# milos-agathon/forge3d

Hardware: AMD Instinct MI355X
Metric: Msamples/s (W*H*spp/s) at 1920x1080, 11616 spp (8 spp/frame x 1452 frames timed); SSIM vs golden (higher is better)
Workload: dtype f32

## Files before the change

forge3d_amd/_native.py:

```python
from __future__ import annotations

import ctypes as C
import os
from pathlib import Path

import numpy as np

_PKG = Path(__file__).resolve().parent
LIB_PATH = _PKG / "libf3dhip.so"

STATUS_OK, STATUS_VALUE, STATUS_RENDER, STATUS_UPLOAD, STATUS_DEVICE = 0, 1, 2, 3, 4
ABI_VERSION = 6
FRAMES_IN_FLIGHT_AUTO = 0xFFFFFFFF

_EARTH = {"flat": 0, "sphere": 1, "ellipsoid": 2, "wgs84": 2}
_REFRACTION = {"none": 0, "bennett": 1, "saemundsson": 2, "effective_radius": 3}


class Desc(C.Structure):
    _fields_ = [
        ("struct_size", C.c_uint32),
        ("heights", C.c_void_p), ("dem_width", C.c_uint32), ("dem_height", C.c_uint32),
        ("spacing_x", C.c_float), ("spacing_z", C.c_float), ("exaggeration", C.c_float),
        ("albedo", C.c_float * 3),
# ... 181 lines not shown


DRAPE_NEAREST, DRAPE_BILINEAR = 0, 1
DRAPE_DEVICE_POINTERS, DRAPE_NO_WAIT, DRAPE_PATCH = 4, 8, 16
DRAPE_MAX_SIDE = 16384
DRAPE_TEXEL_MAX = 65504.0


_P = C.POINTER
ABI = [
    ("f3d_terrain_ref_render", C.c_int, [_P(Desc), _P(Out), C.c_char_p, C.c_size_t]),
    ("f3d_session_create", C.c_int, [_P(Desc), _P(SessionOpts), _P(C.c_void_p), C.c_char_p, C.c_size_t]),
    ("f3d_session_destroy", None, [C.c_void_p]),
    ("f3d_session_enqueue_frames", C.c_int, [C.c_void_p, C.c_uint32, C.c_uint32, C.c_int32, C.c_char_p, C.c_size_t]),
    ("f3d_session_enqueue_trace", C.c_int, [C.c_void_p, C.c_uint32, C.c_uint32, C.c_char_p, C.c_size_t]),
    ("f3d_session_enqueue_merge", C.c_int, [C.c_void_p, C.c_uint32, C.c_int32, C.c_char_p, C.c_size_t]),
    ("f3d_session_set_accumulation", C.c_int, [C.c_void_p, C.c_void_p, C.c_char_p, C.c_size_t]),
    ("f3d_session_halo_export", C.c_int, [C.c_void_p, _P(HaloExport), C.c_char_p, C.c_size_t]),
    ("f3d_session_halo_connect", C.c_int, [C.c_void_p, C.c_int32, _P(HaloExport), C.c_char_p, C.c_size_t]),
    ("f3d_session_halo_probe", C.c_int, [C.c_void_p, C.c_int32, C.c_uint32, _P(C.c_uint32), C.c_char_p, C.c_size_t]),
    ("f3d_session_halo_status", C.c_int, [C.c_void_p, _P(C.c_uint32), C.c_char_p, C.c_size_t]),
    ("f3d_session_halo_stats", C.c_int, [C.c_void_p, _P(HaloStats), C.c_char_p, C.c_size_t]),
    ("f3d_session_enqueue_batch_strip", C.c_int, [C.c_void_p, C.c_uint32, C.c_uint32, C.c_int32, C.c_char_p, C.c_size_t]),
    ("f3d_session_frames_in_flight", C.c_uint32, [C.c_void_p]),
    ("f3d_session_retraced_pixels", C.c_int, [C.c_void_p, _P(C.c_uint64)]),
    ("f3d_session_trace_batch", C.c_uint32, [C.c_void_p, C.c_uint32, C.c_uint32]),
    ("f3d_session_window_stats", C.c_int, [C.c_void_p, _P(C.c_float), _P(C.c_int32), C.c_char_p, C.c_size_t]),
    ("f3d_scene_cache_limit", None, [C.c_uint32]),
    ("f3d_scene_cache_entries", C.c_uint32, []),
    ("f3d_wavefront_render", C.c_int, [C.c_void_p, C.c_uint32, C.c_uint32, C.c_uint32, C.c_uint32, C.c_uint32, C.c_int32,
                                       C.c_void_p, C.c_char_p, C.c_size_t]),
    ("f3d_aether_bake", C.c_int, [C.c_void_p, C.c_void_p, C.c_void_p, C.c_void_p, C.c_void_p, C.c_void_p, _P(C.c_double),
                                  C.c_char_p, C.c_size_t]),
    ("f3d_smoke_render", C.c_int, [C.c_void_p, C.c_void_p, C.c_void_p, C.c_void_p, _P(C.c_double), C.c_char_p, C.c_size_t]),
    ("f3d_smoke_step", C.c_int, [C.c_void_p, C.c_void_p, C.c_void_p, C.c_uint32, C.c_uint32, _P(C.c_double), C.c_char_p, C.c_size_t]),
    ("f3d_aether_reference_render", C.c_int, [C.c_void_p, C.c_void_p, C.c_char_p, C.c_size_t]),
    ("f3d_smoke_composite", C.c_int, [C.c_void_p, C.c_void_p, _P(C.c_double), C.c_char_p, C.c_size_t]),
    ("f3d_session_fingerprint", C.c_int, [C.c_void_p, C.c_void_p, C.c_uint32]),
    ("f3d_session_mesh_tree", C.c_int, [C.c_void_p, _P(C.c_uint32), C.c_void_p, C.c_size_t, C.c_void_p, C.c_size_t, C.c_char_p, C.c_size_t]),
    ("f3d_session_rearm", C.c_int, [C.c_void_p, _P(RearmDesc), C.c_char_p, C.c_size_t]),
    ("f3d_session_render", C.c_int, [C.c_void_p, _P(Out), C.c_char_p, C.c_size_t]),
    ("f3d_session_reaim", C.c_int, [C.c_void_p, _P(ReaimDesc), C.c_char_p, C.c_size_t]),
    ("f3d_session_remesh", C.c_int, [C.c_void_p, _P(RemeshDesc), C.c_char_p, C.c_size_t]),
    ("f3d_session_reterrain", C.c_int, [C.c_void_p, _P(ReterrainDesc), C.c_char_p, C.c_size_t]),
    ("f3d_session_query", C.c_int, [C.c_void_p, _P(QueryDesc), C.c_char_p, C.c_size_t]),
    ("f3d_session_raster", C.c_int, [C.c_void_p, _P(RasterDesc), C.c_char_p, C.c_size_t]),
    ("f3d_session_horizon", C.c_int, [C.c_void_p, _P(HorizonDesc), C.c_char_p, C.c_size_t]),
    ("f3d_session_irradiation", C.c_int, [C.c_void_p, _P(IrradiationDesc), C.c_char_p, C.c_size_t]),
    ("f3d_session_clearance", C.c_int, [C.c_void_p, _P(ClearanceDesc), C.c_char_p, C.c_size_t]),
    ("f3d_session_drape", C.c_int, [C.c_void_p, _P(DrapeDesc), C.c_char_p, C.c_size_t]),
    ("f3d_session_draped", C.c_int, [C.c_void_p, _P(C.c_uint32)]),
    ("f3d_session_certificates", C.c_int, [C.c_void_p, _P(C.c_uint64)]),
    ("f3d_session_sky_blocks", C.c_int, [C.c_void_p, _P(C.c_uint32)]),
    ("f3d_session_debug_wave_times", C.c_int, [C.c_void_p, C.c_void_p]),
    ("f3d_session_halo", C.c_int, [C.c_void_p, C.c_int32, C.c_int32, _P(C.c_void_p), _P(C.c_uint64)]),
    ("f3d_session_resolve", C.c_int, [C.c_void_p, C.c_uint32, C.c_void_p, C.c_void_p, C.c_void_p, C.c_void_p,
                                      _P(C.c_int32), C.c_char_p, C.c_size_t]),
    ("f3d_session_resolve_device", C.c_int, [C.c_void_p, C.c_uint32, C.c_void_p, C.c_void_p, C.c_void_p,
                                             C.c_void_p, C.c_char_p, C.c_size_t]),
    ("f3d_session_setup_ms", C.c_int, [C.c_void_p, _P(C.c_double), C.c_uint32]),
    ("f3d_session_info", C.c_int, [C.c_void_p, _P(C.c_uint64), _P(C.c_uint64), _P(C.c_uint64), _P(C.c_uint32),
                                   _P(C.c_uint32)]),
    ("f3d_session_kernel_timing", C.c_int, [C.c_void_p, C.c_int32, _P(C.c_double), _P(C.c_uint32)]),
    ("f3d_session_sample_lanes", C.c_uint32, [C.c_void_p]),
    ("f3d_session_row_costs", C.c_int, [C.c_void_p, _P(C.c_float), C.c_uint32, C.c_char_p, C.c_size_t]),
    ("f3d_session_primary_start", C.c_void_p, [C.c_void_p]),
    ("f3d_smoke_set_stream", None, [C.c_void_p]),
    ("f3d_smoke_wait_fields_read", C.c_int, [C.c_void_p]),
    ("f3d_smoke_seq_create", C.c_int, [C.c_void_p, C.c_void_p, _P(C.c_void_p), C.c_char_p, C.c_size_t]),
    ("f3d_smoke_seq_destroy", None, [C.c_void_p]),
    ("f3d_smoke_seq_streams", C.c_int, [C.c_void_p, _P(C.c_void_p), _P(C.c_void_p)]),
    ("f3d_smoke_seq_step", C.c_int, [C.c_void_p, C.c_void_p, C.c_void_p, C.c_void_p, C.c_uint32, C.c_uint32, _P(C.c_double), C.c_char_p, C.c_size_t]),
    ("f3d_smoke_seq_render", C.c_int, [C.c_void_p, C.c_void_p, C.c_void_p, C.c_void_p, C.c_void_p, _P(C.c_double), C.c_char_p, C.c_size_t]),
    ("f3d_smoke_seq_composite", C.c_int, [C.c_void_p, C.c_void_p, C.c_void_p, _P(C.c_double), C.c_char_p, C.c_size_t]),
    ("f3d_smoke_seq_stats", C.c_int, [C.c_void_p, C.c_void_p, C.c_char_p, C.c_size_t]),
    ("f3d_halo_rows", C.c_uint32, []),
    ("f3d_session_enqueue_frame_part", C.c_int, [C.c_void_p, C.c_uint32, C.c_uint32, C.c_int32, C.c_char_p, C.c_size_t]),
    ("f3d_atrous_denoise", C.c_int, [C.c_void_p, C.c_void_p, C.c_void_p, C.c_void_p, C.c_uint32, C.c_uint32, C.c_int32,
                                     C.c_float, C.c_float, C.c_float, C.c_float, C.c_void_p, C.c_char_p, C.c_size_t]),
    ("f3d_build_minmax_mips", C.c_int, [C.c_void_p, C.c_uint32, C.c_uint32, C.c_void_p, C.c_void_p, C.c_uint32,
                                        _P(C.c_uint64), C.c_char_p, C.c_size_t]),
    ("f3d_terrain_trace_batch", C.c_int, [C.c_void_p, C.c_uint32, C.c_uint32, C.c_float, C.c_float, C.c_float,
                                          C.c_float, C.c_float, C.c_float, C.c_uint32, C.c_void_p, C.c_uint32,
                                          C.c_int32, C.c_int32, C.c_void_p, C.c_void_p, C.c_void_p, C.c_char_p,
                                          C.c_size_t]),
    ("f3d_effective_radius_m", C.c_int, [C.c_int32, C.c_double, C.c_double, C.c_int32, C.c_double, C.c_double,
                                         C.c_double, C.c_double, _P(C.c_double), C.c_char_p, C.c_size_t]),
    ("f3d_device_count", C.c_int, []),
    ("f3d_device_name", C.c_char_p, [C.c_int32]),
    ("f3d_version", C.c_char_p, []),
    ("f3d_abi_version", C.c_uint32, []),
    ("f3d_device_pool_trim", None, []),
    ("f3d_source_digest", C.c_char_p, []),
    ("f3d_debug_poison", None, [C.c_int32]),
]

_lib = None


def library_path() -> Path:
    return Path(os.environ.get("F3D_HIP_LIBRARY", str(LIB_PATH)))


HIPCC_FLAGS = [
    "--offload-arch=gfx950", "-O3", "-std=c++17", "-fPIC", "-shared",
    "-ffp-contract=off",
    "-fno-slp-vectorize",
]
KERNEL_FLAGS = [
]
HIP_SOURCES = ["f3d_kernels.hip", "f3d_host.hip", "f3d_denoise.hip", "f3d_smoke.hip", "f3d_smoke_sim.hip", "f3d_composite.hip", "f3d_lbvh.hip", "f3d_bvh_refit.hip", "f3d_retable.hip", "f3d_wavefront.hip",
               "f3d_aether_bake.hip", "f3d_aether_ref.hip"]


def source_digest() -> str:
    import hashlib

    csrc, inc = _PKG / "csrc", _PKG.parent / "include"
    if not csrc.is_dir() or not inc.is_dir():
        return None
    h = hashlib.sha256(" ".join(HIPCC_FLAGS + KERNEL_FLAGS + HIP_SOURCES).encode())
    for f in sorted(csrc.glob("*.h")) + sorted(csrc.glob("*.hip")) + sorted(inc.glob("*.h")):
        h.update(f.name.encode())
        h.update(f.read_bytes())
    return h.hexdigest()[:16]


def _hipcc() -> str:
    import shutil

    for cand in (os.environ.get("HIPCC"), shutil.which("hipcc"), "/opt/rocm/bin/hipcc"):
        if cand and Path(cand).exists():
            return cand
    raise RuntimeError("hipcc not found (expected /opt/rocm/bin/hipcc)")
# ... 267 lines not shown
```

forge3d_amd/csrc/f3d_build.h:

```cpp
#pragma once

#include "f3d_scene.h"

namespace f3d {

struct PyramidBuildParams {
    const float *heights;
    uint32_t w, h;
    float exaggeration;
    LeafRec *leaves;
    uint32_t leaf_tiles_x, leaf_dim_x, leaf_dim_y;
};

struct LevelBuildParams {
    const LeafRec *leaves;
    const NodeRec *src;
    NodeRec *dst;
    uint32_t level;
    uint32_t src_w, src_h;
    uint32_t dst_w, dst_h;
    uint32_t src_tiles_x, dst_tiles_x;
    uint32_t dst_dim_x, dst_dim_y;
    uint32_t cell_w, cell_h;
};

struct BandBuildParams {
    const LeafRec *leaves;
    const NodeRec *src;
    NodeRec *dst;
    uint32_t level;
    uint32_t width, height;
    uint32_t shift;
    uint32_t src_tiles_x;
    uint32_t cell_w, cell_h;
};

F3D_HD float min4(const LeafRec &h) { return f_min(f_min(f_min(h.h00, h.h10), h.h01), h.h11); }
F3D_HD float max4(const LeafRec &h) { return f_max(f_max(f_max(h.h00, h.h10), h.h01), h.h11); }

F3D_HD void leaf_build_at(const PyramidBuildParams &B, uint32_t x, uint32_t y) {
    LeafRec rec{0.0f, 0.0f, 0.0f, 0.0f};
    if (x + 1u < B.w && y + 1u < B.h) {
        const size_t i = (size_t)y * B.w + x;
        rec.h00 = B.heights[i] * B.exaggeration;
        rec.h10 = B.heights[i + 1] * B.exaggeration;
        rec.h01 = B.heights[i + B.w] * B.exaggeration;
        rec.h11 = B.heights[i + B.w + 1] * B.exaggeration;
    }
    B.leaves[tiled_index(x, y, B.leaf_tiles_x)] = rec;
}

F3D_HD void level_build_at(const LevelBuildParams &B, uint32_t x, uint32_t y) {
    float mn = __builtin_inff(), mx = -__builtin_inff();
    if (x < B.dst_w && y < B.dst_h) {
        for (uint32_t dy = 0u; dy < 2u; dy++) {
            for (uint32_t dx = 0u; dx < 2u; dx++) {
                uint32_t sx = 2u * x + dx, sy = 2u * y + dy;
                sx = sx < B.src_w - 1u ? sx : B.src_w - 1u;
                sy = sy < B.src_h - 1u ? sy : B.src_h - 1u;
                if (B.level == 1u) {
                    if (sx < B.cell_w && sy < B.cell_h) {
                        const LeafRec h = B.leaves[tiled_index(sx, sy, B.src_tiles_x)];
                        mn = f_min(mn, min4(h));
                        mx = f_max(mx, max4(h));
                    }
                } else {
                    const NodeRec s = B.src[tiled_index(sx, sy, B.src_tiles_x)];
                    mn = f_min(mn, s.mn);
                    mx = f_max(mx, s.mx);
                }
            }
        }
    }
    B.dst[tiled_index(x, y, B.dst_tiles_x)] = NodeRec{mn, mx};
}

F3D_HD void band_build_at(const BandBuildParams &B, uint32_t x, uint32_t z) {
    NodeRec out{__builtin_inff(), -__builtin_inff()};
    if (B.level == 0u) {
        if (x < B.cell_w && z < B.cell_h) {
            const LeafRec h = B.leaves[tiled_index(x, z, B.src_tiles_x)];
            out = NodeRec{min4(h), max4(h)};
        }
    } else {
        out = B.src[tiled_index(x, z, B.src_tiles_x)];
    }
    B.dst[((size_t)z << B.shift) + x] = out;
}

}
```

forge3d_amd/csrc/f3d_frame.h:

```cpp
#pragma once
#include "f3d_launch.h"
#include "f3d_shade.h"
#include "f3d_query.h"
#include "f3d_raster.h"
#include "f3d_horizon.h"
#include "f3d_irradiation.h"
#include "f3d_clearance.h"
#include "f3d_lds.h"
#include "f3d_tiles.h"
#include "f3d_skyblocks.h"

namespace f3d {

template <uint32_t S = 1u>
__device__ __forceinline__ bool tile_pixel(const FrameParams &P, uint32_t &gx, uint32_t &gy, uint32_t &tile,
                                           const uint32_t *order = nullptr, uint32_t wg = 0xFFFFFFFFu) {
    if (wg == 0xFFFFFFFFu) wg = blockIdx.x;
    constexpr TileDims shape = tile_shape<S>();
    const uint32_t rows = P.band_end - P.band_begin;
    const TileGrid grid = tile_grid(P.cam.width, rows, shape);
    if (!workgroup_tile(wg, grid, P.tile_map, order, tile)) return false;
    tile_lane_pixel(tile, threadIdx.x, grid.tiles_x, P.band_begin, shape, gx, gy);
    return gx < P.cam.width && gy < P.band_end;
}
// ... 382 lines not shown
            if (used == have_n) {
                if (++k == kWfChunk) {
                    if (!next_chunk(lane)) return false;
                } else {
                    used = 0u;
                    have_n = (uint32_t)__shfl((int)my_count, (int)k, kWave);
                }
                continue;
            }
            const uint32_t give = have_n - used < n_idle - given ? have_n - used : n_idle - given;
            if (was_idle && rank >= given && rank < given + give) {
                const uint32_t j = used + (rank - given);
                const size_t slot = (size_t)(chunk * kWfChunk + k) * kWfRegion + (W.kind == 1u ? kWfRegion - 1u - j : j);
                const float4 o = W.ray_o[slot];
                V3 d = W.dir;
                if (SUN) {
                    t_stop = W.ray_stop[slot];
                } else {
                    const float4 dd = W.ray_d[slot];
                    d = V3{dd.x, dd.y, dd.z};
                    t_stop = dd.w;
                }
                tag = f_bits(o.w);
                r = make_ray(W.terrain, V3{o.x, o.y, o.z}, 1e-3f, d, 1e30f, SUN);
                have = true;
            }
            used += give;
            given += give;
        }
        return true;
    }
    __device__ __forceinline__ void verdict(uint32_t tag, bool blocked) const {
        if (!blocked) return;
        float4 *rec = W.trace + 2u * (size_t)tag + (SUN ? 0u : 1u);
        float4 v = *rec;
        if (SUN) *rec = float4{(v.x * 0.0f) * 1.0f, (v.y * 0.0f) * 1.0f, (v.z * 0.0f) * 1.0f, v.w};
        else *rec = float4{v.x * 0.0f, v.y * 0.0f, v.z * 0.0f, v.w};
    }
};
template <bool SUN, int MIN_WAVES>
__global__ __launch_bounds__(kWave, MIN_WAVES) void k_wf_occl(const WfOcclParams W) {
    constexpr uint32_t kRows = kFifoWords * kLeafFifoRows;
    __shared__ __attribute__((aligned(16))) uint32_t lds[kRows * kWave + 4 * kMaxLevels];
    LdsPending pend = make_pending(lds, W.terrain, kRows);
    WfSource<SUN> src{W, 0u, (W.regions + kWfChunk - 1u) / kWfChunk, 0u, 0u, 0u, 0u, true};
    march_stream<SUN>(W.terrain, src, pend, W.quorum ? W.quorum : (uint32_t)F3D_STREAM_QUORUM);
}

__device__ __forceinline__ void batch_slot(uint32_t &frame_in_batch, uint32_t &slot) {
    const uint32_t linear = blockIdx.y * gridDim.x + blockIdx.x, group = linear / kNumXcd, xcd = linear % kNumXcd;
    frame_in_batch = group % gridDim.y;
    slot = (group / gridDim.y) * kNumXcd + xcd;
}
template <int MIN_WAVES, uint32_t S, bool MESH = false>
__global__ __launch_bounds__(kWave, MIN_WAVES) void k_trace(const FrameParams P) {
    __shared__ __attribute__((aligned(16))) uint32_t lds[kLdsWords];
    const unsigned long long t_start = wall_clock64();
    typename PendingFor<MESH>::type pend{make_pending(lds, P.terrain)};
    uint32_t gx = 0u, gy = 0u, tile, frame_in_batch, slot;
    batch_slot(frame_in_batch, slot);
    const bool active = tile_pixel<S>(P, gx, gy, tile, P.tile_order, slot);
    trace_lanes<S>(P, P.frame_index + frame_in_batch, tile, active, pend);
    if (lane_now() == 0u && frame_in_batch == 0u && P.tile_cost && tile != 0xFFFFFFFFu)
        P.tile_cost[tile] = (uint32_t)(wall_clock64() - t_start);
}

__global__ __launch_bounds__(kWave) void k_merge(const FrameParams P) {
    __shared__ __attribute__((aligned(16))) uint32_t lds[kLdsWords];
    uint32_t gx = 0u, gy = 0u;
    const bool active = tile_pixel(P, gx, gy);
    float m2 = 0.0f;
    const size_t pixels = (size_t)(P.row_end - P.row_begin) * P.cam.width;
    const size_t lp = active ? (size_t)(gy - P.row_begin) * P.cam.width + gx : 0u;
    const float4 *rec = P.trace + 2u * ((size_t)(P.frame_index - P.trace_first) * P.spp * pixels + lp);
    bool redo = false;
    if (active) {
        const FrameHead h = frame_head<true>(P, gx, gy);
        if (P.same_sun == 0u && P.frame_index > 0u) P.head[lp].y = h.prev_valid ? kHeadPrevValid : 0u;
        if (P.spp == 8u) {
            m2 = merge_pixel_n<8u>(P, gx, gy, h, rec, pixels, P.same_sun == 0u, redo);
        } else {
            if (P.same_sun == 0u) redo = merge_mispredicted(P, h, rec, pixels);
            if (!redo) m2 = merge_pixel(P, gx, gy, h, rec, pixels);
        }
    }
    if (__ballot(redo) != 0ull) {
        LdsPending pend = make_pending(lds, P.terrain);
        if (redo) {
            m2 = fix_pixel(P, gx, gy, rec, pixels, pend);
            atomicAdd(&P.fix_count[2], 1u);
        }
    }
    if (P.collect_stats != 0u) publish_window_stats(P, active, m2);
}

__global__ __launch_bounds__(kWave) void k_trace_init(const FrameParams P) {
    uint32_t gx, gy;
    if (!tile_pixel(P, gx, gy)) return;
    const size_t lp = (size_t)(gy - P.row_begin) * P.cam.width + gx;
    P.head[lp] = first_head(P, P.gbuffer_n[lp]);
}

__device__ __forceinline__ bool head_neighbourhood_empty(const FrameParams &P, uint32_t gx, uint32_t gy) {
    const uint32_t lane = lane_now();
    const uint32_t x0 = gx - (lane & 7u), y0 = gy - (lane >> 3);
    const uint32_t x_last = (x0 + 7u < P.cam.width ? x0 + 7u : P.cam.width - 1u), y_last = (y0 + 7u < P.band_end ? y0 + 7u : P.band_end - 1u);
    const uint32_t xa = x0 >= kSpatialReachLo ? x0 - kSpatialReachLo : 0u, ya = y0 >= kSpatialReachLo ? y0 - kSpatialReachLo : 0u;
    static_assert(8u + kSpatialReachLo + kSpatialReachHi <= 16u, "the 16 x 16 raster below covers the tile's reach");
    static_assert(kSkyBlockMargin >= kSpatialReachLo && kSkyBlockMargin >= kSpatialReachHi, "a deep-sky block's margin covers the spatial pass");
    const uint32_t xb = x_last + kSpatialReachHi < P.cam.width ? x_last + kSpatialReachHi : P.cam.width - 1u;
    const uint32_t yb = y_last + kSpatialReachHi < P.cam.height ? y_last + kSpatialReachHi : P.cam.height - 1u;
    const uint32_t *words = reinterpret_cast<const uint32_t *>(P.res_in);
    uint32_t some = 0u;
#pragma unroll
    for (uint32_t i = 0u; i < 4u; i++) {
        const uint32_t k = lane + 64u * i, bx = xa + (k & 15u), by = ya + (k >> 4);
        if (bx <= xb && by <= yb) some |= words[4u * reservoir_index(P, bx, by) + 1u] & ~kLightTypeBit;
    }
    return __ballot(some != 0u) == 0ull;
}

__global__ __launch_bounds__(kWave) void k_head(const FrameParams P) {
    uint32_t gx, gy, tile;
    const bool active = tile_pixel<1u>(P, gx, gy, tile);
    if (tile == 0xFFFFFFFFu) return;
    if (P.sky_blocks != nullptr && (P.sky_blocks[tile] & kSkyBlockDeep) != 0u) {
        float m2 = 0.0f;
        if (active) m2 = frame_tail_accumulate(P, gx, gy, all_miss_radiance(P));
        if (P.collect_stats != 0u) publish_window_stats(P, active, m2);
        return;
    }
#if !defined(F3D_NO_EMPTY_HEAD)
    if (P.frame_index > 0u && head_neighbourhood_empty(P, gx, gy)) {
        if (active) {
            const size_t ri = reservoir_index(P, gx, gy), lp = (size_t)(gy - P.row_begin) * P.cam.width + gx;
            const PackedReservoir self = P.res_in[ri];
            P.res_out[ri] = PackedReservoir{0.0f, self.m_lt, 0.0f, self.target_pdf};
            FrameHead h;
            h.centre_hit = P.gbuffer_n[lp].w != 0.0f;
            h.prev_valid = false;
            h.reuse_w = 1.0f;
            h.rng = 0u;
            P.head[lp] = pack_head(h);
        }
        return;
    }
#endif
    if (active) P.head[(size_t)(gy - P.row_begin) * P.cam.width + gx] = pack_head(frame_head<true>(P, gx, gy));
}

template <uint32_t S, bool MESH, bool DRAPE>
__device__ __forceinline__ void frame_wave(const FrameParams &P, uint32_t *lds) {
    const unsigned long long t_start = wall_clock64();
    uint32_t gx = 0u, gy = 0u, tile;
    const bool active = tile_pixel<S>(P, gx, gy, tile, P.tile_order);
    if constexpr (S != 1u) {
        if (P.sky_blocks != nullptr && tile != kNoTile) {
            constexpr TileDims shape = tile_shape<S>();
            const uint32_t block = sky_block_of_tile(tile, tiles_across(P.cam.width, shape), shape, tiles_across(P.cam.width, kSkyBlockShape));
            if ((P.sky_blocks[block] & kSkyBlockDeep) != 0u) return;
        }
    }
    typename PendingFor<MESH>::type pend{make_pending(lds, P.terrain)};
    float m2 = 0.0f;
    if constexpr (S == 1u) {
        if (active) m2 = frame_pixel<DRAPE>(P, gx, gy, pend);
        if (P.collect_stats != 0u) publish_window_stats(P, active, m2);
    } else {
        m2 = frame_lanes<S, DRAPE>(P, tile, active, pend);
        if (P.collect_stats != 0u) publish_window_stats(P, active && (lane_now() & (S - 1u)) == 0u, m2);
    }
    if (lane_now() == 0u) {
        const unsigned long long t_end = wall_clock64();
        if (P.tile_cost && tile != 0xFFFFFFFFu) P.tile_cost[tile] = (uint32_t)(t_end - t_start);
#if defined(F3D_WAVE_TIMES)
        if (P.wave_times) {
            P.wave_times[2u * blockIdx.x] = t_start;
            P.wave_times[2u * blockIdx.x + 1u] = t_end;
        }
#endif
    }
}
template <int VARIANT, int MIN_WAVES = 1, uint32_t S = 1u, bool MESH = false>
__global__ __launch_bounds__(kWave, MIN_WAVES) void k_frame(const FrameParams P) {
    __shared__ __attribute__((aligned(16))) uint32_t lds[kLdsWords];
    frame_wave<S, MESH, false>(P, lds);
}
template <int MIN_WAVES, uint32_t S, bool MESH>
__global__ __launch_bounds__(kWave, MIN_WAVES) void k_frame_drape(const FrameParams P) {
    __shared__ __attribute__((aligned(16))) uint32_t lds[kLdsWords];
    frame_wave<S, MESH, true>(P, lds);
}

struct SkyBlocksParams {
    const uint2 *primary_start;
    uint32_t *blocks;
    SkyBlockGeom geom;
    uint32_t enabled;
};
__global__ __launch_bounds__(kWave) void k_sky_blocks(const SkyBlocksParams B) {
    const uint32_t block = blockIdx.x;
    const auto certified = [&](uint32_t x, uint32_t y) {
        return certified_sky(B.primary_start[(size_t)(y - B.geom.row_begin) * B.geom.width + x]);
    };
    bool clear = false, own = false;
    if (B.primary_start != nullptr) {
        if (B.enabled != 0u) clear = sky_block_lane_clear(B.geom, block, threadIdx.x, certified);
        const uint32_t x = (block % tiles_across(B.geom.width, kSkyBlockShape)) * 8u + (threadIdx.x & 7u);
        const uint32_t y = B.geom.row_begin + (block / tiles_across(B.geom.width, kSkyBlockShape)) * 8u + (threadIdx.x >> 3);
        own = x < B.geom.width && y < B.geom.row_end && certified(x, y);
    }
    const bool deep = __ballot(!clear) == 0ull;
    const uint32_t count = (uint32_t)__popcll(__ballot(own));
    if (threadIdx.x == 0u) B.blocks[block] = (deep ? kSkyBlockDeep : 0u) | (count << kSkyBlockCountShift);
}

__global__ __launch_bounds__(kWave) void k_gbuffer(const FrameParams P, float4 *gbuffer_n, float *depth) {
    __shared__ __attribute__((aligned(16))) uint32_t lds[kLdsWords];
    LdsPending pend = make_pending(lds, P.terrain);
    uint32_t gx, gy;
    if (tile_pixel(P, gx, gy)) gbuffer_pixel(P, gx, gy, gbuffer_n, depth, pend);
}

__global__ __launch_bounds__(kWave) void k_rearm(const RearmParams R) {
    const FrameParams &P = R.frame;
    uint32_t gx, gy;
    if (!tile_pixel(P, gx, gy)) return;
    rearm_certificate(P, gx, gy, P.gbuffer_n, R.depth);
    rearm_clear(R, gx, gy);
    rearm_head(P, gx, gy, P.gbuffer_n[(size_t)(gy - P.row_begin) * P.cam.width + gx]);
}

__global__ __launch_bounds__(kWave) void k_reaim(const RearmParams R) {
    __shared__ __attribute__((aligned(16))) uint32_t lds[kLdsWords];
    LdsPending pend = make_pending(lds, R.frame.terrain);
    uint32_t gx, gy;
    if (tile_pixel(R.frame, gx, gy)) reaim_pixel(R, gx, gy, pend);
}

__global__ __launch_bounds__(kWave) void k_resolve(const ResolveParams R) {
    uint32_t gx, gy;
    const bool active = tile_pixel(R.frame, gx, gy);
    uint32_t flags = 0u;
    if (active) flags = resolve_pixel(R.frame, R.frames, gx, gy, R.rgba, R.albedo, R.normal, &R.aether, R.depth);
    const unsigned long long valid = __ballot((flags & 1u) != 0u), bad = __ballot((flags & 2u) != 0u);
    if (threadIdx.x == 0) {
        if (valid) atomicOr(&R.frame.stats[2], 1u);
        if (bad) atomicOr(&R.frame.stats[3], 1u);
    }
}

__global__ __launch_bounds__(kWave) void k_resolve_drape(const ResolveParams R) {
    uint32_t gx, gy;
    const bool active = tile_pixel(R.frame, gx, gy);
    uint32_t flags = 0u;
    if (active) flags = resolve_pixel<true>(R.frame, R.frames, gx, gy, R.rgba, R.albedo, R.normal, &R.aether, R.depth);
    const unsigned long long valid = __ballot((flags & 1u) != 0u), bad = __ballot((flags & 2u) != 0u);
    if (threadIdx.x == 0) {
        if (valid) atomicOr(&R.frame.stats[2], 1u);
        if (bad) atomicOr(&R.frame.stats[3], 1u);
    }
}

__global__ __launch_bounds__(256) void k_drape_pack(const DrapePackParams B) {
    const uint32_t c = blockIdx.x * 256u + threadIdx.x, r = blockIdx.y;
    if (c < B.cols && r < B.rows) drape_pack_at(B, r, c);
}

__global__ __launch_bounds__(kWave) void k_ray_batch(const RayBatchParams B) {
    __shared__ __attribute__((aligned(16))) uint32_t lds[kLdsWords];
    LdsPending pend = make_pending(lds, B.terrain);
    const uint32_t i = blockIdx.x * kWave + threadIdx.x;
    if (i >= B.n) return;
    const float4 a = B.rays[2 * i], b = B.rays[2 * i + 1];
    const RayCtx r = make_ray(B.terrain, V3{a.x, a.y, a.z}, a.w, V3{b.x, b.y, b.z}, b.w, B.apply_curvature != 0u);
    TraceHit h;
    if (B.any_hit >= 2u) {
        h = march_ray(B.terrain, r, B.any_hit == 2u, B.start_in_cell != 0u, pend);
    } else {
        h = trace_terrain(B.terrain, r, B.any_hit != 0u, pend);
    }
    B.out_hit[i] = h.hit ? 1u : 0u;
    if (B.out_t) B.out_t[i] = h.t;
    if (B.out_normal) {
        B.out_normal[3 * i + 0] = h.hit ? h.n.x : 0.0f;
        B.out_normal[3 * i + 1] = h.hit ? h.n.y : 0.0f;
        B.out_normal[3 * i + 2] = h.hit ? h.n.z : 0.0f;
    }
}

template <bool MESH>
__global__ __launch_bounds__(kWave) void k_query(const QueryParams Q) {
    __shared__ __attribute__((aligned(16))) uint32_t lds[kLdsWords];
    typename PendingFor<MESH>::type pend{make_pending(lds, Q.frame.terrain)};
    const uint32_t i = blockIdx.x * kWave + threadIdx.x;
    if (i < Q.count) query_lane(Q, i, pend);
}

template <bool MESH>
__global__ __launch_bounds__(kWave) void k_raster(const RasterParams R) {
    __shared__ __attribute__((aligned(16))) uint32_t lds[kLdsWords];
    typename PendingFor<MESH>::type pend{make_pending(lds, R.frame.terrain)};
    const uint32_t total = R.rows * R.cols, n = blockIdx.x * kWave + threadIdx.x;
    const size_t words = ((size_t)total + 63u) >> 6;
    const bool have = n < total;
    const V3 o = have ? raster_origin(R, n) : V3{0.0f, 0.0f, 0.0f};
    uint32_t seen = 0u;
    for (uint32_t k = 0u; k < R.target_count; k++) {
        const float4 target = R.targets ? R.targets[k] : float4{R.frame.light.wi.x, R.frame.light.wi.y, R.frame.light.wi.z, 0.0f};
        bool visible = false;
        if (have) visible = raster_visible(R, o, target, pend);
        const unsigned long long word = __ballot(visible);
        if (R.masks && threadIdx.x == 0u) R.masks[(size_t)k * words + blockIdx.x] = word;
        seen += visible ? 1u : 0u;
    }
    if (R.count && have) R.count[n] = seen;
}

struct HorizonLevels {
    const uint32_t *table;
    __device__ __forceinline__ void band_entry(const TerrainDev &, uint32_t level, uint32_t &offset, uint32_t &shift) const {
        const uint2 e = *reinterpret_cast<const uint2 *>(table + 2u * level);
        offset = e.x;
        shift = e.y;
    }
};
__global__ __launch_bounds__(kWave) void k_horizon(const HorizonParams R) {
    __shared__ __attribute__((aligned(8))) uint32_t table[2 * kMaxLevels];
    if (threadIdx.x < kMaxLevels) {
        table[2u * threadIdx.x] = R.terrain.band_offset[threadIdx.x];
        table[2u * threadIdx.x + 1u] = R.terrain.band_shift[threadIdx.x];
// ... 49 lines not shown
        if (R.height) R.height[(size_t)k * total + n] = L;
        lowest = f_min(lowest, L);
    }
    if (R.lowest) R.lowest[n] = lowest;
}

template <bool MESH>
__global__ __launch_bounds__(kWave) void k_irradiation(const IrradiationParams R) {
    __shared__ __attribute__((aligned(16))) uint32_t lds[kLdsWords];
    typename PendingFor<MESH>::type pend{make_pending(lds, R.frame.terrain)};
    const uint32_t total = R.rows * R.cols, n = blockIdx.x * kWave + threadIdx.x;
    const bool have = n < total;
    uint32_t i = 0u, j = 0u;
    const V3 o = have ? irradiation_origin(R, n, i, j) : V3{0.0f, 0.0f, 0.0f};
    const IrradiationSlope s = have ? irradiation_slope(R, i, j) : IrradiationSlope{0.0f, 0.0f, 1.0f};
    float sum = 0.0f;
    uint32_t seen = 0u;
    for (uint32_t k = 0u; k < R.direction_count; k++) {
        const float4 dir = R.directions[k];
        bool lit = false;
        float term = 0.0f;
        if (have) term = irradiation_term(R, o, s, dir, pend, lit);
        if (lit) {
            sum = sum + term;
            seen += 1u;
        }
    }
    if (!have) return;
    if (R.energy) R.energy[n] = sum;
    if (R.count) R.count[n] = seen;
    if (R.normal) {
        const V3 nrm = irradiation_normal(s);
        R.normal[3u * (size_t)n] = nrm.x;
        R.normal[3u * (size_t)n + 1u] = nrm.y;
        R.normal[3u * (size_t)n + 2u] = nrm.z;
    }
}

__global__ void k_leaf_build(const PyramidBuildParams B) {
    const uint32_t x = blockIdx.x * blockDim.x + threadIdx.x, y = blockIdx.y * blockDim.y + threadIdx.y;
    if (x < B.leaf_dim_x && y < B.leaf_dim_y) leaf_build_at(B, x, y);
}

__global__ void k_band_build(const BandBuildParams B) {
    const uint32_t x = blockIdx.x * blockDim.x + threadIdx.x, z = blockIdx.y * blockDim.y + threadIdx.y;
    if (x < B.width && z < B.height) band_build_at(B, x, z);
}

__global__ void k_level_build(const LevelBuildParams B) {
    const uint32_t x = blockIdx.x * blockDim.x + threadIdx.x, y = blockIdx.y * blockDim.y + threadIdx.y;
    if (x < B.dst_dim_x && y < B.dst_dim_y) level_build_at(B, x, y);
}

struct HorizonBuildParams {
    TerrainDev terrain;
    uint32_t level, bx, bz;
    float *table;
};
__global__ __launch_bounds__(kWave) void k_horizon_build(const HorizonBuildParams B) {
    const uint32_t tiles_x = (B.bx + 7u) >> 3;
    const uint32_t x = (blockIdx.x % tiles_x) * 8u + (threadIdx.x & 7u), z = (blockIdx.x / tiles_x) * 8u + (threadIdx.x >> 3);
    if (x >= B.bx || z >= B.bz) return;
    float out[kIblSectors];
    horizon_block_build(B.terrain, B.level, x, z, out);
    float4 *dst = reinterpret_cast<float4 *>(B.table + ((size_t)z * B.bx + x) * kIblSectors);
    dst[0] = float4{out[0], out[1], out[2], out[3]};
    dst[1] = float4{out[4], out[5], out[6], out[7]};
}

}
```

forge3d_amd/csrc/f3d_host.hip:

```cpp
#include <hip/hip_runtime.h>

#include <atomic>
#include <deque>
#include <exception>
#include <memory>
#include <map>
#include <mutex>
#include <new>
#include <unordered_map>

#include <unistd.h>

#include "f3d_bvh_refit.h"
#include "f3d_devmem.h"
#include "f3d_launch.h"
#include "f3d_lbvh.h"
#include "f3d_meshgrid.h"
#include "f3d_retable.h"
#include "f3d_setup.h"
#include "f3d_tables.h"
#include "f3d_tiles.h"
#include "f3d_skyblocks.h"

using namespace f3d;
// ... 22 lines not shown
    try {
        body();
    } catch (const Failure &f) {
        return report(f, err, errlen);
    } catch (const std::exception &e) {
        if (err && errlen) snprintf(err, errlen, "host failure: %s", e.what());
        return F3D_STATUS_DEVICE;
    } catch (...) {
        if (err && errlen) snprintf(err, errlen, "unknown host failure");
        return F3D_STATUS_DEVICE;
    }
    return F3D_STATUS_OK;
}
f3d_session &checked(f3d_session *s) {
    if (!s) fail(F3D_STATUS_VALUE, "null session handle");
    return *s;
}

}

#include "f3d_host_mem.h"

struct f3d_session {
    double setup_ms[kSetupPhases] = {};
    Ledger mem;
    hipStream_t stream = nullptr;
    int device = 0;
    FrameParams params{};
    std::shared_ptr<CachedTables> scene;
    std::shared_ptr<CachedMesh> mesh;
    uint64_t mesh_counted = 0;
    uint32_t mesh_builder = 0;
    bool mesh_grid = false;
    struct OwnMesh {
        float4 *vertices = nullptr, *tris = nullptr;
        void *nodes = nullptr;
        uint32_t *parent = nullptr, *counter = nullptr;
        int *bounds = nullptr;
        size_t vertex_bytes = 0, tri_bytes = 0, node_bytes = 0, link_bytes = 0 , bounds_bytes = 0;
        uint32_t refits = 0;
        bool live = false;
        uint64_t bytes() const { return (uint64_t)vertex_bytes + tri_bytes + node_bytes + 2u * link_bytes + bounds_bytes; }
        void release(Ledger &mem) {
            mem.free(vertices, vertex_bytes);
            mem.free(tris, tri_bytes);
            mem.free(nodes, node_bytes);
            mem.free(parent, link_bytes);
            mem.free(counter, link_bytes);
            mem.free(bounds, bounds_bytes);
            *this = OwnMesh{};
        }
    } own_mesh;
    uint64_t scene_counted = 0;
    struct OwnTerrain {
        LeafRec *leaves = nullptr;
        NodeRec *bands = nullptr;
        float *staging = nullptr;
        size_t leaf_bytes = 0, band_bytes = 0, staging_bytes = 0;
        bool live = false;
    } own_terrain;
    void *query_scratch = nullptr;
    uint64_t query_bytes = 0;
    size_t query_capacity = 0;
    void *raster_scratch = nullptr;
    uint64_t raster_bytes = 0;
    struct Drape {
        void *buffer = nullptr;
        uint64_t bytes = 0;
        uint32_t rows = 0, cols = 0;
        DrapeDev record{};
        float *staging = nullptr;
        uint64_t staging_bytes = 0;
    } drape;
    TerrainTables tables;
    uint32_t width = 0, height = 0, row_begin = 0, row_end = 0, rows = 0;
    PackedReservoir *res[2] = {nullptr, nullptr};
    float4 *gbuffer_n = nullptr;
    float *depth = nullptr;
    uint32_t *stats = nullptr;
    uint32_t *host_stats = nullptr;
    uint32_t *halo_flags = nullptr;
    uint32_t halo_frames_published = 0;
    unsigned long long halo_timeout_ticks = 0;
    double wall_clock_khz = 100000.0;
    struct PeerLink {
        void *opened[3] = {nullptr, nullptr, nullptr};
        const PackedReservoir *res[2] = {nullptr, nullptr};
        const uint32_t *flags = nullptr;
        uint32_t rows = 0;
        bool connected = false;
    } peer[2];
    bool owns_reservoirs = false;
    uint8_t *d_rgba = nullptr;
    float *d_albedo = nullptr, *d_normal = nullptr;
    int variant = 0;
    AetherDev aether{};
    bool require_valid_reservoirs = false;
    f3d_terrain_ref_desc desc{};
    bool rendered = false;
    double reaim_seconds = 0.0;
    uint64_t budget = 0;
    struct Band {
        uint32_t begin = 0, end = 0;
        hipStream_t stream = nullptr;
        bool edge = true;
        hipEvent_t done[2] = {nullptr, nullptr};
// ... 373 lines not shown
#if !defined(F3D_NO_PRIMARY_START)
    P.primary_start = (uint2 *)s.mem.alloc(px * sizeof(uint2), "primary-ray certificates");
#endif
#if !defined(F3D_NO_SUN_CLEAR)
    P.sun_clear = (float2 *)s.mem.alloc(px * sizeof(float2), "sun-ray certificates");
#endif
    s.depth = (float *)s.mem.alloc(px * sizeof(float), "depth AOV");
    s.d_rgba = (uint8_t *)s.mem.alloc(px * 4, "rgba8 output");
    s.d_albedo = (float *)s.mem.alloc(px * 3 * sizeof(float), "albedo AOV");
    s.d_normal = (float *)s.mem.alloc(px * 3 * sizeof(float), "normal AOV");
    if (opts && opts->ext_stats) s.stats = (uint32_t *)opts->ext_stats;
    else s.stats = (uint32_t *)s.mem.alloc(4 * sizeof(uint32_t), "stats");
    hip_check(hipMemsetAsync(P.accum_mean, 0, px * sizeof(float4), s.stream), "accum clear");
    hip_check(hipMemsetAsync(P.welford_m2, 0, px * sizeof(float), s.stream), "welford clear");
    hip_check(hipMemsetAsync(s.stats, 0, 4 * sizeof(uint32_t), s.stream), "stats clear");
    hip_check(hipHostMalloc((void **)&s.host_stats, 4 * sizeof(uint32_t), hipHostMallocDefault), "pinned stats");
    s.mem.note_host_visible(4 * sizeof(uint32_t));
    P.gbuffer_n = s.gbuffer_n;
    P.stats = s.stats;
    clock.lap(kSetupAlloc);

    if (s.mem.device_bytes > s.budget)
        fail(F3D_STATUS_RENDER,
             "terrain PT exceeds the memory budget before rendering: tracked total %llu (host-visible %llu) > limit %llu",
             (unsigned long long)s.mem.device_bytes, (unsigned long long)s.mem.host_visible_peak,
             (unsigned long long)s.budget);

    plan_bands(s, opts ? opts->bands : 0u, opts ? opts->band_streams : 0u);
    const bool lpt = s.bands.size() == 1 && ((s.variant / 1000) % 10 == 0);
    if ((s.variant / 1000) % 10 == 4) P.tile_map = 2u;
    if (lpt) {
        uint32_t grid = 0;
        const uint32_t tiles = frame_tile_count(P, &grid);
        s.tile_cost = (uint32_t *)s.mem.alloc((size_t)tiles * sizeof(uint32_t), "tile costs");
        s.tile_order = (uint32_t *)s.mem.alloc((size_t)(grid ? grid : 1u) * sizeof(uint32_t), "tile order");
        hip_check(hipMemsetAsync(s.tile_cost, 0, (size_t)tiles * sizeof(uint32_t), s.stream), "tile cost clear");
    }

    P.frame_index = 0;
    P.res_in = s.res[1];
    P.res_out = s.res[0];
    P.collect_stats = 0;
    hip_check(launch_gbuffer(P, s.gbuffer_n, s.depth, s.stream), "g-buffer pass");
    if (const size_t bytes = (size_t)std::max(sky_block_count(P), 1u) * sizeof(uint32_t); sky_blocks_wanted(s) && s.mem.device_bytes + bytes <= s.budget) {
        s.sky_blocks = (uint32_t *)s.mem.alloc(bytes, "deep-sky blocks");
        enqueue_sky_blocks(s);
    }
    if (s.fd_frames) {
        P.band_begin = s.row_begin;
        P.band_end = s.row_end;
        hip_check(launch_trace_init(P, s.stream), "trace prediction init");
    }
    clock.lap(kSetupPasses);
}

template <class Launch>
void ordered_timed_launch(f3d_session &s, hipStream_t stream, uint32_t frame, Launch &&launch) {
    constexpr int64_t kOrderEvery = 4;
    FrameParams &P = s.params;
    P.tile_cost = s.tile_cost;
    P.tile_order = nullptr;
    if (s.tile_cost && s.cost_frame >= 0) {
        if (s.order_frame < 0 || s.cost_frame - s.order_frame >= kOrderEvery) {
            hip_check(launch_tile_order(P, s.tile_cost, s.tile_order, stream), "tile order kernel");
            s.order_frame = s.cost_frame;
        }
        P.tile_order = s.tile_order;
    }
    hipEvent_t e0 = nullptr, e1 = nullptr;
    if (s.timing) {
        hip_check(hipEventCreate(&e0), "event");
        hip_check(hipEventCreate(&e1), "event");
        hip_check(hipEventRecord(e0, stream), "event record");
    }
    launch();
    if (s.tile_cost) s.cost_frame = (int64_t)frame;
    P.tile_order = nullptr;
    P.tile_cost = nullptr;
    if (s.timing) {
        hip_check(hipEventRecord(e1, stream), "event record");
        s.events.emplace_back(e0, e1);
    }
}

void enqueue_band(f3d_session &s, f3d_session::Band &b, size_t index, uint32_t frame, bool collect) {
    FrameParams &P = s.params;
    P.frame_index = frame;
    P.res_out = s.res[frame & 1u];
    P.res_in = s.res[(frame & 1u) ^ 1u];
    P.collect_stats = collect ? 1u : 0u;
    P.band_begin = b.begin;
    P.band_end = b.end;
    const bool piped = b.stream != s.stream;
    if (b.last != (int64_t)frame - 1 && !(b.last < 0 && frame == 0u) && piped)
        fail(F3D_STATUS_VALUE, "frames must be enqueued in order (band %zu is at frame %lld, frame %u wanted)", index,
             (long long)b.last, frame);
    if (piped) {
        hip_check(hipStreamWaitEvent(b.stream, s.fork, 0), "band fork");
        for (int d = -1; d <= 1; d += 2) {
            const size_t n = index + (size_t)d;
            if (n >= s.bands.size() || frame == 0u) continue;
            f3d_session::Band &nb = s.bands[n];
            if (nb.last != (int64_t)frame - 1 && nb.last != (int64_t)frame)
                fail(F3D_STATUS_VALUE, "frames must be enqueued in order (band %zu is at frame %lld, frame %u wanted)", n,
                     (long long)nb.last, frame);
            if (nb.stream != b.stream) hip_check(hipStreamWaitEvent(b.stream, nb.done[(frame - 1u) & 1u], 0), "band wait");
// ... 424 lines not shown
uint32_t f3d_session_sample_lanes(f3d_session *s) { return s ? s->params.sample_lanes : 0u; }
const void *f3d_session_primary_start(f3d_session *s) {
    if (!s || !(s->params.cam.cone_delta >= 0.0f) || !s->params.primary_start) return nullptr;
    DeviceGuard guard(s->device);
    if (hipStreamSynchronize(s->stream) != hipSuccess) return nullptr;
    return s->params.primary_start;
}

int f3d_session_row_costs(f3d_session *s, float *out, uint32_t rows, char *err, size_t errlen) {
    try {
        if (!s || !out) fail(F3D_STATUS_VALUE, "null argument");
        if (rows != s->rows) fail(F3D_STATUS_VALUE, "the session owns %u rows, %u asked for", s->rows, rows);
        if (!s->tile_cost || s->cost_frame < 0) fail(F3D_STATUS_VALUE, "no frame has left its tile costs yet (a one-band session with the default tile map does, from its first fused frame on)");
        DeviceGuard guard(s->device);
        hip_check(hipStreamSynchronize(s->stream), "row costs");
        FrameParams P = s->params;
        P.band_begin = s->row_begin;
        P.band_end = s->row_end;
        const uint32_t tiles = frame_tile_count(P, nullptr);
        std::vector<uint32_t> cost(tiles);
        hip_check(hipMemcpy(cost.data(), s->tile_cost, (size_t)tiles * sizeof(uint32_t), hipMemcpyDeviceToHost), "tile costs");
        spread_tile_costs(cost.data(), s->width, rows, tile_shape(sample_lanes_of(P)), out);
        return F3D_STATUS_OK;
    } catch (const Failure &f) {
        return report(f, err, errlen);
    }
}
uint32_t f3d_halo_rows(void) { return kHaloRows; }

int f3d_session_fingerprint(f3d_session *s, uint64_t *out, uint32_t count) {
    if (!s || !out || count < 16u) return F3D_STATUS_VALUE;
    try {
        DeviceGuard guard(s->device);
        hip_check(hipStreamSynchronize(s->stream), "fingerprint");
        for (auto &b : s->bands)
            if (b.stream) hip_check(hipStreamSynchronize(b.stream), "fingerprint");
        const FrameParams &P = s->params;
        auto dev = [&](const void *p, size_t bytes) -> uint64_t {
            if (!p || !bytes) return 0ull;
            std::vector<uint8_t> host(bytes);
            hip_check(hipMemcpy(host.data(), p, bytes, hipMemcpyDeviceToHost), "fingerprint download");
            return hash_bytes(host.data(), bytes, 0x243F6A8885A308D3ull);
        };
        const TableLayout &L = s->scene ? s->scene->tables.layout : s->tables.layout;
        const size_t px = (size_t)s->rows * s->width, res_n = (size_t)(s->rows + 2u * kHaloRows) * s->width;
        TerrainDev t = P.terrain;
        t.leaves = nullptr;
        t.nodes = nullptr;
        t.bands = nullptr;
        t.horizon = nullptr;
        t.mesh_bands = nullptr;
        t.mesh_cell_start = nullptr;
        t.mesh_cell_tris = nullptr;
        MeshDev m = P.mesh;
        m.vertices = nullptr;
        m.indices = nullptr;
        m.bvh_nodes = nullptr;
        m.bvh_tris = nullptr;
        m.bvh4_nodes = nullptr;
        const uint32_t scalars[8] = {P.spp, P.row_begin, P.row_end, P.tile_map, P.sample_lanes, P.same_sun, P.env.width, P.env.height};
        out[0] = hash_bytes(&P.cam, sizeof(P.cam), 1);
        out[1] = hash_bytes(&P.light, sizeof(P.light), 2);
        out[2] = hash_bytes(&t, sizeof(t), 3);
        out[3] = hash_bytes(&m, sizeof(m), 4);
        out[4] = hash_bytes(scalars, sizeof(scalars), 5) ^ hash_bytes(&P.env.intensity, sizeof(float), 6);
        out[5] = dev(P.terrain.leaves, L.leaf_count * sizeof(LeafRec));
        out[6] = dev(P.terrain.bands, L.band_count * sizeof(NodeRec));
        out[7] = dev(P.mesh.vertices, (size_t)P.mesh.vertex_count * sizeof(float4));
        out[8] = dev(P.mesh.indices, (size_t)P.mesh.index_count * sizeof(uint32_t));
        out[9] = P.mesh.bvh4_nodes ? dev(P.mesh.bvh4_nodes, (size_t)P.mesh.bvh4_node_count * sizeof(Bvh4Node))
                                   : dev(P.mesh.bvh_nodes, (size_t)P.mesh.bvh_node_count * sizeof(BvhNode));
        out[10] = dev(P.mesh.bvh_tris, (size_t)P.mesh.index_count * sizeof(float4));
        out[11] = dev(P.env.texels, (size_t)P.env.width * P.env.height * sizeof(float4));
        out[12] = dev(s->gbuffer_n, px * sizeof(float4));
        out[13] = dev(s->res[0], res_n * sizeof(PackedReservoir)) ^ (dev(s->res[1], res_n * sizeof(PackedReservoir)) * 3ull);
        out[14] = dev(P.accum_mean, px * sizeof(float4)) ^ (dev(P.welford_m2, px * sizeof(float)) * 3ull);
        out[15] = dev(P.head, P.head ? px * sizeof(uint2) : 0);
        if (count >= 17u) {
            DrapeDev rec = s->drape.record;
            rec.texels = nullptr;
            out[16] = s->drape.buffer ? hash_bytes(&rec, sizeof(rec), 7) ^ (dev((const char *)s->drape.buffer + sizeof(DrapeDev), (size_t)s->drape.bytes - sizeof(DrapeDev)) * 3ull) : 0ull;
        }
        return F3D_STATUS_OK;
    } catch (...) {
        return F3D_STATUS_DEVICE;
    }
}

int f3d_session_mesh_tree(f3d_session *s, uint32_t info[4], void *nodes, size_t node_capacity_bytes, void *tris, size_t tri_capacity_bytes,
                          char *err, size_t errlen) {
    return c_abi(err, errlen, [&] {
        DeviceGuard g(checked(s).device);
        if (!info) fail(F3D_STATUS_VALUE, "null info record");
        hip_check(hipStreamSynchronize(s->stream), "mesh tree");
        for (auto &b : s->bands)
            if (b.stream) hip_check(hipStreamSynchronize(b.stream), "mesh tree");
        const MeshDev &M = s->params.mesh;
        const uint32_t form = M.bvh4_nodes ? 2u : (M.bvh_nodes ? 1u : 0u);
        const void *d_nodes = form == 2u ? (const void *)M.bvh4_nodes : (const void *)M.bvh_nodes;
        const uint32_t node_count = form == 2u ? M.bvh4_node_count : (form == 1u ? M.bvh_node_count : 0u);
        const size_t record = form == 2u ? sizeof(Bvh4Node) : sizeof(BvhNode);
        const size_t owner_tri_bytes = s->own_mesh.live ? s->own_mesh.tri_bytes : (s->mesh ? s->mesh->tri_bytes : 0);
        const size_t tri_count = form != 0u && M.bvh_tris ? owner_tri_bytes / (3u * sizeof(float4)) : 0u;
        info[0] = form;
        info[1] = node_count;
        info[2] = (uint32_t)tri_count;
        info[3] = 0u;
        const size_t node_bytes = (size_t)node_count * record, tri_bytes = tri_count * 3u * sizeof(float4);
        if (nodes && node_capacity_bytes < node_bytes)
            fail(F3D_STATUS_VALUE, "the node buffer holds %zu bytes, the tree has %u records of %zu bytes: %zu", node_capacity_bytes, node_count,
                 record, node_bytes);
        if (tris && tri_capacity_bytes < tri_bytes)
            fail(F3D_STATUS_VALUE, "the triangle buffer holds %zu bytes, the tree has %zu triangles of 48 bytes: %zu", tri_capacity_bytes,
                 tri_count, tri_bytes);
        if (nodes && node_bytes) hip_check(hipMemcpy(nodes, d_nodes, node_bytes, hipMemcpyDeviceToHost), "mesh tree nodes");
        if (tris && tri_bytes) hip_check(hipMemcpy(tris, M.bvh_tris, tri_bytes, hipMemcpyDeviceToHost), "mesh tree triangles");
    });
}

int f3d_session_render(f3d_session *s, f3d_terrain_ref_out *out, char *err, size_t errlen) {
    return c_abi(err, errlen, [&] {
        DeviceGuard g(checked(s).device);
        if (!out) fail(F3D_STATUS_VALUE, "null output record");
        const double t_setup = now_s();
        hip_check(hipStreamSynchronize(s->stream), "setup sync");
        out->setup_seconds = now_s() - t_setup + s->reaim_seconds;
        s->reaim_seconds = 0.0;
        render_loop(*s, out);
    });
}

int f3d_session_certificates(f3d_session *s, uint64_t out[2]) {
    if (!s || !out) return F3D_STATUS_VALUE;
    try {
        DeviceGuard guard(s->device);
        join_bands(*s);
        hip_check(hipStreamSynchronize(s->stream), "certificates");
        const size_t px = (size_t)s->rows * s->width;
        auto dev = [&](const void *ptr, size_t bytes) -> uint64_t {
            if (!ptr || !bytes) return 0ull;
            std::vector<uint8_t> host(bytes);
            hip_check(hipMemcpy(host.data(), ptr, bytes, hipMemcpyDeviceToHost), "certificate download");
            return hash_bytes(host.data(), bytes, 0x243F6A8885A308D3ull);
        };
        out[0] = dev(s->params.sun_clear, px * sizeof(float2));
        out[1] = dev(s->params.primary_start, px * sizeof(uint2));
        return F3D_STATUS_OK;
    } catch (...) {
        return F3D_STATUS_DEVICE;
    }
}

int f3d_session_sky_blocks(f3d_session *s, uint32_t out[4]) {
    if (!s || !out) return F3D_STATUS_VALUE;
    try {
        DeviceGuard guard(s->device);
        join_bands(*s);
        hip_check(hipStreamSynchronize(s->stream), "sky blocks");
        FrameParams P = s->params;
        P.row_begin = s->row_begin;
        P.row_end = s->row_end;
        const uint32_t blocks = sky_block_count(P), blocks_x = tiles_across(s->width, kSkyBlockShape);
        out[0] = blocks;
        out[1] = out[2] = out[3] = 0u;
        if (!s->sky_blocks || blocks == 0u) return F3D_STATUS_OK;
        std::vector<uint32_t> words(blocks);
        hip_check(hipMemcpy(words.data(), s->sky_blocks, (size_t)blocks * sizeof(uint32_t), hipMemcpyDeviceToHost), "sky-block download");
        const bool in_use = sky_blocks_in_use(*s);
        for (uint32_t b = 0; b < blocks; b++) {
            out[2] += words[b] >> kSkyBlockCountShift;
            if (in_use && (words[b] & kSkyBlockDeep) != 0u) {
                const uint32_t x0 = (b % blocks_x) * 8u, y0 = (b / blocks_x) * 8u;
                out[1]++;
                out[3] += std::min(8u, s->width - x0) * std::min(8u, s->rows - y0);
            }
        }
        return F3D_STATUS_OK;
    } catch (...) {
        return F3D_STATUS_DEVICE;
    }
}

int f3d_session_debug_wave_times(f3d_session *s, void *device_buffer) {
#if defined(F3D_WAVE_TIMES)
    if (!s) return F3D_STATUS_VALUE;
    s->params.wave_times = (unsigned long long *)device_buffer;
    return F3D_STATUS_OK;
#else
    (void)s;
    (void)device_buffer;
    return F3D_STATUS_VALUE;
#endif
}

int f3d_terrain_ref_render(const f3d_terrain_ref_desc *desc, f3d_terrain_ref_out *out, char *err, size_t errlen) {
    if (err && errlen) err[0] = 0;
    if (!desc || !out) return F3D_STATUS_VALUE;
    f3d_session *s = new (std::nothrow) f3d_session();
    if (!s) return F3D_STATUS_DEVICE;
    int rc = F3D_STATUS_OK;
    try {
        const double t_setup = now_s();
        f3d_session_opts one_shot{};
        one_shot.struct_size = (uint32_t)sizeof(one_shot);
// ... 31 lines not shown
            fail(F3D_STATUS_DEVICE, "no HIP device available: libf3dhip has no CPU fallback");
        float *d_h = (float *)mem.alloc(n * sizeof(float), "DEM upload");
        hip_check(hipMemcpy(d_h, heights, n * sizeof(float), hipMemcpyHostToDevice), "DEM upload");
        TerrainTables t = build_tables(mem, d_h, width, height, 1.0f, nullptr, true);
        hip_check(hipDeviceSynchronize(), "table build");
        const TableLayout &L = t.layout;
        const uint32_t levels = L.levels;
        uint64_t tot = 0;
        for (uint32_t l = 0; l < levels; l++) tot += (uint64_t)L.level_w[l] * L.level_h[l] * 2;
        if (total_floats) *total_floats = tot;
        if (dims_out)
            for (uint32_t l = 0; l < levels && l < max_levels; l++) {
                dims_out[2 * l] = L.level_w[l];
                dims_out[2 * l + 1] = L.level_h[l];
            }
        if (levels_out) {
            std::vector<LeafRec> leaves(L.leaf_count);
            std::vector<NodeRec> nodes(L.node_count ? L.node_count : 1);
            hip_check(hipMemcpy(leaves.data(), t.leaves, L.leaf_count * sizeof(LeafRec), hipMemcpyDeviceToHost), "readback");
            if (L.node_count)
                hip_check(hipMemcpy(nodes.data(), t.nodes, L.node_count * sizeof(NodeRec), hipMemcpyDeviceToHost), "readback");
            uint64_t off = 0;
            for (uint32_t l = 0; l < levels; l++) {
                for (uint32_t y = 0; y < L.level_h[l]; y++)
                    for (uint32_t x = 0; x < L.level_w[l]; x++) {
                        float mn, mx;
                        if (l == 0) {
                            if (x < t.dev.cell_w && y < t.dev.cell_h) {
                                const LeafRec &h = leaves[tiled_index(x, y, t.dev.tiles_x[0])];
                                mn = min4(h);
                                mx = max4(h);
                            } else {
                                mn = INFINITY;
                                mx = -INFINITY;
                            }
                        } else {
                            const NodeRec &r = nodes[t.dev.node_offset[l] + tiled_index(x, y, t.dev.tiles_x[l])];
                            mn = r.mn;
                            mx = r.mx;
                        }
                        levels_out[off++] = mn;
                        levels_out[off++] = mx;
                    }
            }
        }
        rc = (int)levels;
    } catch (const Failure &f) {
        rc = -report(f, err, errlen);
    }
    mem.release();
    return rc;
}

int f3d_terrain_trace_batch(const float *heights, uint32_t width, uint32_t height, float origin_x, float origin_z,
                            float spacing_x, float spacing_z, float exaggeration, float inv_two_r_prime,
                            uint32_t curvature_enabled, const float *rays, uint32_t n, int32_t any_hit,
                            int32_t apply_curvature, uint32_t *out_hit, float *out_t, float *out_normal, char *err,
                            size_t errlen) {
    if (err && errlen) err[0] = 0;
    Ledger mem;
    int rc = F3D_STATUS_OK;
    try {
        if (width < 2 || height < 2)
            fail(F3D_STATUS_UPLOAD, "terrain heightfield must be at least 2x2 texels, got %ux%u", width, height);
        int ndev = 0;
        if (hipGetDeviceCount(&ndev) != hipSuccess || ndev <= 0)
            fail(F3D_STATUS_DEVICE, "no HIP device available: libf3dhip has no CPU fallback");
        const size_t dem_n = (size_t)width * height;
        float *d_h = (float *)mem.alloc(dem_n * sizeof(float), "DEM upload");
        hip_check(hipMemcpy(d_h, heights, dem_n * sizeof(float), hipMemcpyHostToDevice), "DEM upload");
        TerrainTables t = build_tables(mem, d_h, width, height, exaggeration, nullptr, true);
        RayBatchParams B{};
        B.terrain = t.dev;
        B.terrain.origin_x = origin_x;
        B.terrain.origin_z = origin_z;
        B.terrain.spacing_x = spacing_x;
        B.terrain.spacing_z = spacing_z;
        B.terrain.inv_spacing_x = 1.0f / spacing_x;
        B.terrain.inv_spacing_z = 1.0f / spacing_z;
        B.terrain.inv_two_r_prime = inv_two_r_prime;
        B.terrain.curvature_enabled = curvature_enabled;
        float4 *d_rays = (float4 *)mem.alloc((size_t)n * 32, "rays");
        hip_check(hipMemcpy(d_rays, rays, (size_t)n * 32, hipMemcpyHostToDevice), "ray upload");
        B.rays = d_rays;
        B.n = n;
        B.any_hit = (uint32_t)any_hit & 3u;
        B.start_in_cell = ((uint32_t)any_hit >> 2) & 1u;
        B.terrain.share_below = ((uint32_t)any_hit >> 8) & 255u;
        B.apply_curvature = apply_curvature != 0;
        B.out_hit = (uint32_t *)mem.alloc((size_t)n * 4, "hits");
        B.out_t = (float *)mem.alloc((size_t)n * 4, "t");
        B.out_normal = (float *)mem.alloc((size_t)n * 12, "normals");
        hip_check(launch_ray_batch(B, nullptr), "ray batch kernel");
        hip_check(hipDeviceSynchronize(), "ray batch");
        hip_check(hipMemcpy(out_hit, B.out_hit, (size_t)n * 4, hipMemcpyDeviceToHost), "readback");
        if (out_t) hip_check(hipMemcpy(out_t, B.out_t, (size_t)n * 4, hipMemcpyDeviceToHost), "readback");
        if (out_normal) hip_check(hipMemcpy(out_normal, B.out_normal, (size_t)n * 12, hipMemcpyDeviceToHost), "readback");
    } catch (const Failure &f) {
        rc = report(f, err, errlen);
    }
    mem.release();
    return rc;
}

int f3d_effective_radius_m(int32_t earth_model, double latitude_deg, double sphere_radius_m, int32_t refraction_model,
                           double pressure_mbar, double temperature_c, double refraction_k, double azimuth_deg,
                           double *radius_out, char *err, size_t errlen) {
    if (err && errlen) err[0] = 0;
    try {
        *radius_out = effective_radius(earth_model, latitude_deg, sphere_radius_m, refraction_model, pressure_mbar,
                                       temperature_c, refraction_k, azimuth_deg);
    } catch (const Failure &f) {
        return report(f, err, errlen);
    }
    return F3D_STATUS_OK;
}

void f3d_scene_cache_limit(uint32_t entries) {
    std::lock_guard<std::mutex> lock(g_scene_mutex);
    g_scene_limit = entries;
    while (g_scene_cache.size() > g_scene_limit) {
        size_t oldest = 0;
        for (size_t i = 1; i < g_scene_cache.size(); i++)
            if (g_scene_cache[i]->stamp < g_scene_cache[oldest]->stamp) oldest = i;
        g_scene_cache.erase(g_scene_cache.begin() + (long)oldest);
    }
    while (g_mesh_cache.size() > g_scene_limit) {
        size_t oldest = 0;
        for (size_t i = 1; i < g_mesh_cache.size(); i++)
            if (g_mesh_cache[i]->stamp < g_mesh_cache[oldest]->stamp) oldest = i;
        g_mesh_cache.erase(g_mesh_cache.begin() + (long)oldest);
    }
}

// ... 35 lines not shown
```

forge3d_amd/csrc/f3d_host_mem.h:

```cpp
#pragma once

namespace f3d {
namespace {
int poison_from_env() {
    const char *v = getenv("F3D_POISON");
    return (v && *v) ? (atoi(v) & 0xFF) : -1;
}
std::atomic<int> g_poison_pattern{poison_from_env()};
std::mutex g_poison_mutex;
std::unordered_map<void *, void *> g_poison_bases;
}
int poison_pattern() { return g_poison_pattern.load(); }

namespace {
struct PoolBlock {
    void *p;
    size_t bytes;
    int device;
};
std::mutex g_pool_mutex;
std::vector<PoolBlock> &g_pool_free = *new std::vector<PoolBlock>();
std::unordered_map<void *, PoolBlock> &g_pool_live = *new std::unordered_map<void *, PoolBlock>();
size_t g_pool_bytes = 0;
size_t pool_limit() {
// ... 116 lines not shown
        Ledger &mem;
        std::vector<std::pair<void *, size_t>> got;
        ~Take() {
            for (auto &g : got) mem.free(g.first, g.second);
        }
        void *operator()(size_t bytes, const char *what) {
            void *p = mem.alloc(bytes, what);
            got.emplace_back(p, bytes);
            return p;
        }
        void commit() { got.clear(); }
    };
};

struct TerrainTables {
    TerrainDev dev{};
    TableLayout layout;
    uint64_t bytes = 0;
    LeafRec *leaves = nullptr;
    NodeRec *nodes = nullptr;
    NodeRec *bands = nullptr;
};

TerrainTables build_tables(Ledger &mem, const float *d_heights, uint32_t w, uint32_t h, float exaggeration,
                           hipStream_t stream, bool keep_nodes) {
    TerrainTables t;
    t.layout = table_layout(w, h);
    const TableLayout &L = t.layout;
    t.leaves = (LeafRec *)mem.alloc(L.leaf_count * sizeof(LeafRec), "leaf table");
    t.nodes = (NodeRec *)mem.alloc((L.node_count ? L.node_count : 1) * sizeof(NodeRec), "node table");
    t.bands = (NodeRec *)mem.alloc(L.band_count * sizeof(NodeRec), "band tables");
    t.bytes = L.leaf_count * sizeof(LeafRec) + (L.node_count + L.band_count) * sizeof(NodeRec);
    hip_check(launch_leaf_build(leaf_build_params(L, d_heights, w, h, exaggeration, t.leaves), stream),
              "leaf table build");
    for (uint32_t l = 1; l < L.levels; l++)
        hip_check(launch_level_build(level_build_params(L, l, t.leaves, t.nodes), stream), "node table build");
    for (uint32_t l = 0; l < L.levels; l++)
        hip_check(launch_band_build(band_build_params(L, l, t.leaves, t.nodes, t.bands), stream), "band table build");
#if !defined(F3D_TRAVERSAL_DESCENT)
    if (!keep_nodes) {
        hip_check(hipStreamSynchronize(stream), "table build");
        mem.free(t.nodes, (L.node_count ? L.node_count : 1) * sizeof(NodeRec));
        t.nodes = nullptr;
        t.bytes = L.leaf_count * sizeof(LeafRec) + L.band_count * sizeof(NodeRec);
    }
#endif
    apply_layout(L, t.dev);
    t.dev.leaves = t.leaves;
    t.dev.nodes = t.nodes;
    t.dev.bands = t.bands;
    return t;
}

}

enum SetupPhase { kSetupTotal = 0, kSetupValidate, kSetupHash, kSetupUpload, kSetupTables, kSetupScene, kSetupAlloc, kSetupPasses, kSetupPhases };
struct SetupClock {
    double *ms;
    std::chrono::steady_clock::time_point t0 = std::chrono::steady_clock::now(), last = t0;
    explicit SetupClock(double *out) : ms(out) {}
    void lap(SetupPhase phase) {
        const auto now = std::chrono::steady_clock::now();
        ms[phase] += std::chrono::duration<double, std::milli>(now - last).count();
        ms[kSetupTotal] = std::chrono::duration<double, std::milli>(now - t0).count();
        last = now;
    }
};
static thread_local double *g_setup_ms = nullptr;

namespace {

struct CachedTables {
    int device = 0;
    uint64_t key = 0, key2 = 0, dem_bytes = 0;
    uint32_t w = 0, h = 0;
    float exaggeration = 0.0f;
    Ledger mem;
    TerrainTables tables;
    uint64_t stamp = 0;
    struct Horizon {
        float spacing_x, spacing_z;
        float *table;
        uint32_t level, bx, bz;
    };
    std::vector<Horizon> horizons;
    ~CachedTables() {
        int prev = -1;
        (void)hipGetDevice(&prev);
        (void)hipSetDevice(device);
        mem.release();
        if (prev >= 0) (void)hipSetDevice(prev);
    }
};

std::mutex g_scene_mutex;
std::vector<std::shared_ptr<CachedTables>> &g_scene_cache = *new std::vector<std::shared_ptr<CachedTables>>();
uint64_t g_scene_stamp = 0;
size_t g_scene_limit = 2;

uint64_t hash_bytes(const void *data, size_t n, uint64_t seed) {
    const uint8_t *p = (const uint8_t *)data;
    uint64_t h = seed ^ (n * 0x9E3779B97F4A7C15ull);
    size_t i = 0;
    for (; i + 8 <= n; i += 8) {
        uint64_t v;
        memcpy(&v, p + i, 8);
        h = (h ^ v) * 0xFF51AFD7ED558CCDull;
        h ^= h >> 32;
    }
    for (; i < n; i++) h = (h ^ p[i]) * 0x100000001B3ull;
    return h ^ (h >> 29);
}

struct StagingPair {
    std::mutex mutex;
    void *buffer[2] = {nullptr, nullptr};
    hipEvent_t drained[2] = {nullptr, nullptr};
};
StagingPair &staging_for_current_device() {
    static std::mutex map_mutex;
    static std::map<int, std::unique_ptr<StagingPair>> &pairs = *new std::map<int, std::unique_ptr<StagingPair>>();
    int device = 0;
    hip_check(hipGetDevice(&device), "current device");
    std::lock_guard<std::mutex> lock(map_mutex);
    std::unique_ptr<StagingPair> &slot = pairs[device];
    if (!slot) slot.reset(new StagingPair());
    return *slot;
}
void upload_staged(void *dst, const void *src, size_t bytes, hipStream_t stream, bool stream_ordered = false) {
    constexpr size_t kChunk = 4u << 20;
    StagingPair &pair = staging_for_current_device();
    std::lock_guard<std::mutex> lock(pair.mutex);
    for (int i = 0; i < 2; i++)
        if (!pair.buffer[i]) {
            hip_check(hipHostMalloc(&pair.buffer[i], kChunk, hipHostMallocPortable), "pinned staging buffer");
            hip_check(hipEventCreateWithFlags(&pair.drained[i], hipEventDisableTiming), "staging event");
        }
    if (bytes < (256u << 10) && !stream_ordered) {
        hip_check(hipMemcpy(dst, src, bytes, hipMemcpyHostToDevice), "upload");
        return;
    }
    size_t done = 0;
// ... 228 lines not shown
```

forge3d_amd/csrc/f3d_host_update.h:

```cpp
#pragma once

namespace {

struct Update {
    f3d_session &s;
    const bool cam;
    const double t_host = now_s();
    f3d_terrain_ref_desc d;
    FrameParams U{};
    bool require_valid = false;

    Update(f3d_session &session, const f3d_session_rearm_desc &r, const f3d_session_reaim_desc *aim, const char *done)
        : s(session), cam(aim != nullptr) {
        if (aim) check_struct_size(*aim, "f3d_session_reaim_desc");
        check_struct_size(r, "f3d_session_rearm_desc");
        if (s.peer[0].connected || s.peer[1].connected)
            fail(F3D_STATUS_VALUE, "a session with peer halos cannot be %s: the frame counters its neighbours poll only rise", done);
        d = s.desc;
        d.sun_azimuth_deg = r.sun_azimuth_deg;
        d.sun_elevation_deg = r.sun_elevation_deg;
        d.sun_intensity = r.sun_intensity;
        for (int c = 0; c < 3; c++) d.sun_color[c] = r.sun_color[c];
        d.exposure = r.exposure;
        d.env_intensity = r.env_intensity;
// ... 23 lines not shown
    }
    void validate() { validate([] {}); }

    void apply() {
        FrameParams &P = s.params;
        P.cam = U.cam;
        P.light = U.light;
        P.terrain.inv_two_r_prime = U.terrain.inv_two_r_prime;
        P.terrain.curvature_enabled = U.terrain.curvature_enabled;
        P.env.intensity = U.env.intensity;
        P.same_sun = same_sun_of(P);
        if (s.aether.enabled) aether_sun_terms(s.aether, d);
        s.require_valid_reservoirs = require_valid;
        s.desc = d;
        s.desc.mesh_vertices = nullptr;
        s.desc.mesh_indices = nullptr;

        join_bands(s);
        P.band_begin = s.row_begin;
        P.band_end = s.row_end;
        P.frame_index = 0;
        P.trace_first = 0u;
        P.res_in = s.res[1];
        P.res_out = s.res[0];
        P.collect_stats = 0;
        P.tile_order = nullptr;
        P.tile_cost = nullptr;
        RearmParams R{};
        R.frame = P;
        R.gbuffer_n = s.gbuffer_n;
        R.depth = s.depth;
        R.res[0] = s.res[0];
        R.res[1] = s.res[1];
        R.tile_cost = s.tile_cost;
        R.tiles = s.tile_cost ? frame_tile_count(P, nullptr) : 0u;
        if (cam) {
            hip_check(launch_reaim(R, s.stream), "re-aim kernel");
            enqueue_sky_blocks(s);
        } else {
            hip_check(launch_rearm(R, s.stream), "re-arm kernel");
        }
        s.cost_frame = s.order_frame = -1;
        s.rendered = false;
        s.trace_first = -1;
        s.trace_count = 0;
        for (auto &b : s.bands) {
            b.last = -1;
            b.unjoined = false;
        }
        s.reaim_seconds = cam ? now_s() - t_host : 0.0;
    }
};

void check_budget(const f3d_session &s, uint64_t planned, const char *update, const char *brings) {
    if (planned > s.budget)
        fail(F3D_STATUS_RENDER, "%s exceeds the memory budget: %s the tracked total to %llu > limit %llu", update, brings,
             (unsigned long long)planned, (unsigned long long)s.budget);
}

void rearm(f3d_session &s, const f3d_session_rearm_desc &r) {
    Update u(s, r, nullptr, "re-armed");
    u.validate();
    u.apply();
}

void reaim(f3d_session &s, const f3d_session_reaim_desc &a) {
    Update u(s, a.arm, &a, "re-aimed");
    u.validate();
    u.apply();
}

void remesh_refit(f3d_session &s, const float *vertices, uint32_t vertex_count) {
    FrameParams &P = s.params;
    f3d_session::OwnMesh &O = s.own_mesh;
    const CachedMesh &E = *s.mesh;
    const bool first = !O.live;
    const uint32_t nodes = E.dev.bvh4_nodes ? E.dev.bvh4_node_count : E.dev.bvh_node_count;
    if (first) {
        f3d_session::OwnMesh N;
        N.vertex_bytes = E.vertex_bytes;
        N.tri_bytes = E.tri_bytes;
        N.node_bytes = E.node_bytes;
        N.link_bytes = (size_t)std::max(nodes, 1u) * sizeof(uint32_t);
        N.bounds_bytes = 12u * sizeof(int);
        check_budget(s, s.mem.device_bytes - s.mesh_counted + E.index_bytes + N.bytes(), "re-mesh",
                     "the session's own copy of the mesh and the refit tables bring");
        Ledger::Take take{s.mem};
        N.vertices = (float4 *)take(N.vertex_bytes, "re-mesh vertices");
        if (N.tri_bytes) N.tris = (float4 *)take(N.tri_bytes, "re-mesh BVH triangles");
        if (N.node_bytes) N.nodes = take(N.node_bytes, "re-mesh BVH nodes");
        N.parent = (uint32_t *)take(N.link_bytes, "re-mesh parent links");
        N.counter = (uint32_t *)take(N.link_bytes, "re-mesh arrival counters");
        N.bounds = (int *)take(N.bounds_bytes, "re-mesh scene bounds");
        take.commit();
        s.mem.device_bytes -= s.mesh_counted;
        s.mesh_counted = E.index_bytes;
        s.mem.device_bytes += s.mesh_counted;
        join_bands(s);
        if (N.tris) hip_check(hipMemcpyAsync(N.tris, E.dev.bvh_tris, N.tri_bytes, hipMemcpyDeviceToDevice, s.stream), "re-mesh copy");
        if (N.nodes)
            hip_check(hipMemcpyAsync(N.nodes, E.dev.bvh4_nodes ? (const void *)E.dev.bvh4_nodes : (const void *)E.dev.bvh_nodes, N.node_bytes,
                                     hipMemcpyDeviceToDevice, s.stream), "re-mesh copy");
        hip_check(hipMemsetAsync(N.counter, 0, N.link_bytes, s.stream), "re-mesh counters");
        static const int kEmptyBounds[12] = {0x7F800000, 0x7F800000, 0x7F800000, (int)0x807FFFFF, (int)0x807FFFFF, (int)0x807FFFFF,
                                             0x7F800000, 0x7F800000, 0x7F800000, (int)0x807FFFFF, (int)0x807FFFFF, (int)0x807FFFFF};
        hip_check(hipMemcpyAsync(N.bounds, kEmptyBounds, sizeof(kEmptyBounds), hipMemcpyHostToDevice, s.stream), "re-mesh bounds");
        N.live = true;
// ... 77 lines not shown
    const uint32_t w = s.desc.dem_width, h = s.desc.dem_height;
    if (!t.heights || t.width == 0u || t.height == 0u)
        fail(F3D_STATUS_VALUE, "re-terrain block is empty (%ux%u samples): a block holds at least one sample", t.width, t.height);
    if (t.x0 >= w || t.y0 >= h || t.width > w - t.x0 || t.height > h - t.y0)
        fail(F3D_STATUS_VALUE, "re-terrain block of %ux%u samples at sample (%u, %u) leaves the session's %ux%u DEM (another DEM size needs a new session)",
             t.width, t.height, t.x0, t.y0, w, h);
    const bool whole = t.x0 == 0u && t.y0 == 0u && t.width == w && t.height == h;
    if (t.exaggeration != 0.0f && !(t.exaggeration == s.desc.exaggeration)) {
        if (!whole)
            fail(F3D_STATUS_VALUE, "a new exaggeration (%g, the session's is %g) rescales every sample: give it with the whole %ux%u DEM, not with a block",
                 (double)t.exaggeration, (double)s.desc.exaggeration, w, h);
        u.d.exaggeration = t.exaggeration;
    }
    const size_t samples = (size_t)t.width * t.height, block_bytes = samples * sizeof(float);
    u.validate([&] {
        uint32_t bad = 0u;
        for (size_t i = 0; i < samples; i++) {
            uint32_t v;
            memcpy(&v, t.heights + i, sizeof v);
            bad |= (uint32_t)((v & 0x7F800000u) == 0x7F800000u);
        }
        if (bad) fail(F3D_STATUS_UPLOAD, "terrain heightfield contains non-finite samples");
    });

    f3d_session::OwnTerrain &O = s.own_terrain;
    const TableLayout &L = s.tables.layout;
    const size_t leaf_bytes = L.leaf_count * sizeof(LeafRec), band_bytes = L.band_count * sizeof(NodeRec);
    const bool take_tables = !O.leaves, grow = block_bytes > O.staging_bytes;
    if (take_tables || grow) {
        char brings[96];
        snprintf(brings, sizeof brings, "the session's own tables and the staging buffer of a %ux%u block bring", t.width, t.height);
        check_budget(s, s.mem.device_bytes - (take_tables ? s.scene_counted : 0u) + (take_tables ? leaf_bytes + band_bytes : 0u) -
                            (grow ? O.staging_bytes : 0u) + (grow ? block_bytes : 0u), "re-terrain", brings);
        f3d_session::OwnTerrain N = O;
        Ledger::Take take{s.mem};
        if (grow) {
            N.staging = (float *)take(block_bytes, "re-terrain staging");
            N.staging_bytes = block_bytes;
        }
        if (take_tables) {
            N.leaves = (LeafRec *)take(leaf_bytes, "re-terrain leaf table");
            N.bands = (NodeRec *)take(band_bytes, "re-terrain band tables");
            N.leaf_bytes = leaf_bytes;
            N.band_bytes = band_bytes;
        }
        take.commit();
        if (grow && O.staging) s.mem.free(O.staging, O.staging_bytes);
        if (take_tables) {
            s.mem.device_bytes -= s.scene_counted;
            s.scene_counted = 0u;
        }
        O = N;
    }
    join_bands(s);
    if (!O.live) {
        hip_check(hipMemcpyAsync(O.leaves, s.tables.leaves, leaf_bytes, hipMemcpyDeviceToDevice, s.stream), "re-terrain copy");
        hip_check(hipMemcpyAsync(O.bands, s.tables.bands, band_bytes, hipMemcpyDeviceToDevice, s.stream), "re-terrain copy");
    }
    upload_staged(O.staging, t.heights, block_bytes, s.stream, true);
    hip_check(launch_retable(retable_params(L, O.staging, t.x0, t.y0, t.width, t.height, u.d.exaggeration, O.leaves, O.bands), s.stream),
              "re-terrain table kernels");
    if (!O.live) {
        O.live = true;
        s.tables.leaves = O.leaves;
        s.tables.bands = O.bands;
        s.tables.dev.leaves = O.leaves;
        s.tables.dev.bands = O.bands;
        s.params.terrain.leaves = O.leaves;
        s.params.terrain.bands = O.bands;
        s.params.terrain.mesh_bands = O.bands;
    }
    u.apply();
}

template <class Desc>
int update_entry(f3d_session *s, const Desc *desc, const char *noun, void (*update)(f3d_session &, const Desc &), char *err, size_t errlen) {
    return c_abi(err, errlen, [&] {
        DeviceGuard g(checked(s).device);
        if (!desc) fail(F3D_STATUS_VALUE, "null %s descriptor", noun);
        update(*s, *desc);
    });
}

}

extern "C" {

int f3d_session_rearm(f3d_session *s, const f3d_session_rearm_desc *desc, char *err, size_t errlen) {
    return update_entry(s, desc, "re-arm", rearm, err, errlen);
}

int f3d_session_reaim(f3d_session *s, const f3d_session_reaim_desc *desc, char *err, size_t errlen) {
    return update_entry(s, desc, "re-aim", reaim, err, errlen);
}

int f3d_session_remesh(f3d_session *s, const f3d_session_remesh_desc *desc, char *err, size_t errlen) {
    return update_entry(s, desc, "re-mesh", remesh, err, errlen);
}

int f3d_session_reterrain(f3d_session *s, const f3d_session_reterrain_desc *desc, char *err, size_t errlen) {
    return update_entry(s, desc, "re-terrain", reterrain, err, errlen);
}

}
```

forge3d_amd/csrc/f3d_kernels.hip:

```cpp
#include <type_traits>

#include "f3d_frame.h"

namespace f3d {

void horizon_table_dims(uint32_t cell_w, uint32_t cell_h, uint32_t *level, uint32_t *bx, uint32_t *bz) {
    *level = horizon_block_level(cell_w, cell_h);
    *bx = (cell_w + (1u << *level) - 1u) >> *level;
    *bz = (cell_h + (1u << *level) - 1u) >> *level;
}
hipError_t launch_horizon_build(const TerrainDev &terrain, float *table, hipStream_t stream) {
    HorizonBuildParams B{};
    B.terrain = terrain;
    B.terrain.horizon = nullptr;
    horizon_table_dims(terrain.cell_w, terrain.cell_h, &B.level, &B.bx, &B.bz);
    B.table = table;
    hipLaunchKernelGGL(k_horizon_build, dim3(((B.bx + 7u) >> 3) * ((B.bz + 7u) >> 3)), dim3(kWave), 0, stream, B);
    return hipGetLastError();
}
static inline TileGrid band_tiles(const FrameParams &p, uint32_t lanes) {
    return tile_grid(p.cam.width, p.band_end - p.band_begin, tile_shape(lanes));
}
static inline uint32_t frame_grid(const FrameParams &p, uint32_t lanes = 1u) { return launch_size(band_tiles(p, lanes), p.tile_map); }

template <class F>
static bool with_lanes(uint32_t lanes, F &&launch) {
    switch (lanes) {
        case 1: launch(std::integral_constant<uint32_t, 1u>{}); return true;
        case 2: launch(std::integral_constant<uint32_t, 2u>{}); return true;
        case 4: launch(std::integral_constant<uint32_t, 4u>{}); return true;
        case 8: launch(std::integral_constant<uint32_t, 8u>{}); return true;
        default: return false;
    }
}
template <class F>
static void with_mesh(bool mesh, F &&launch) {
    if (mesh) launch(std::true_type{});
    else launch(std::false_type{});
}
static inline bool has_mesh(const FrameParams &p) { return p.mesh.traversal_mode == 0u; }

hipError_t launch_head(const FrameParams &p, hipStream_t stream) {
    if (frame_grid(p) == 0u) return hipSuccess;
    hipLaunchKernelGGL(k_head, dim3(frame_grid(p)), dim3(kWave), 0, stream, p);
    return hipGetLastError();
}

#if !defined(F3D_DRAPE_WAVES)
#define F3D_DRAPE_WAVES 5
#endif
constexpr int kDrapeWaves = F3D_DRAPE_WAVES;
hipError_t launch_frame(const FrameParams &p, int variant, hipStream_t stream) {
    const uint32_t lanes = sample_lanes_of(p);
    if (frame_grid(p, lanes) == 0u) return hipSuccess;
    const dim3 grid(frame_grid(p, lanes)), block(kWave);
    static const bool force_mesh = getenv("F3D_FORCE_MESH_KERNEL") != nullptr;
    const bool mesh = has_mesh(p) || force_mesh;
    const int budget = variant % 1000;
    bool known = false;
    if (p.drape) {
        known = budget == 0 && with_lanes(lanes, [&](auto S) {
            with_mesh(mesh, [&](auto M) { hipLaunchKernelGGL((k_frame_drape<kDrapeWaves, S(), M()>), grid, block, 0, stream, p); });
        });
    } else if (budget == 0) {
        known = with_lanes(lanes, [&](auto S) {
            with_mesh(mesh, [&](auto M) { hipLaunchKernelGGL((k_frame<0, 6, S(), M()>), grid, block, 0, stream, p); });
        });
    } else if (budget == 104 && lanes == 1u) {
        known = true;
        with_mesh(mesh, [&](auto M) { hipLaunchKernelGGL((k_frame<0, 4, 1u, M()>), grid, block, 0, stream, p); });
    } else if (budget == 105 && lanes == 4u) {
        known = true;
        with_mesh(mesh, [&](auto M) { hipLaunchKernelGGL((k_frame<0, 5, 4u, M()>), grid, block, 0, stream, p); });
    }
    return known ? hipGetLastError() : hipErrorInvalidValue;
}
hipError_t launch_trace(const FrameParams &p, uint32_t frames, hipStream_t stream) {
    const uint32_t lanes = sample_lanes_of(p);
    if (frame_grid(p, lanes) == 0u || frames == 0u) return hipSuccess;
    const dim3 grid(frame_grid(p, lanes), frames), block(kWave);
    const bool known = with_lanes(lanes, [&](auto S) {
        with_mesh(has_mesh(p), [&](auto M) { hipLaunchKernelGGL((k_trace<6, S(), M()>), grid, block, 0, stream, p); });
    });
    return known ? hipGetLastError() : hipErrorInvalidValue;
}
template <class K>
static uint32_t persistent_grid(K kernel) {
    int device = 0, cus = 256, per_cu = 0;
    (void)hipGetDevice(&device);
    (void)hipDeviceGetAttribute(&cus, hipDeviceAttributeMultiprocessorCount, device);
    if (hipOccupancyMaxActiveBlocksPerMultiprocessor(&per_cu, kernel, kWave, 0) != hipSuccess || per_cu <= 0) per_cu = 16;
    return (uint32_t)cus * (uint32_t)per_cu;
}
hipError_t launch_trace_wavefront(const FrameParams &p, uint32_t frames, uint32_t quorum, hipStream_t stream) {
    const uint32_t lanes = sample_lanes_of(p);
    if (frame_grid(p, lanes) == 0u || frames == 0u) return hipSuccess;
    hipError_t err = hipMemsetAsync(p.wf.cursors, 0, 4u * sizeof(uint32_t), stream);
    if (err != hipSuccess) return err;
    const dim3 grid(frame_grid(p, lanes), frames), block(kWave);
    if (!with_lanes(lanes, [&](auto S) { hipLaunchKernelGGL((k_wf_primary<6, S()>), grid, block, 0, stream, p); }))
        return hipErrorInvalidValue;
    static const uint32_t sun_grid = persistent_grid(k_wf_occl<true, 7>), ibl_grid = persistent_grid(k_wf_occl<false, 8>);
    WfOcclParams W{};
    W.terrain = p.terrain;
    W.trace = p.trace;
    W.counts = p.wf.counts;
    W.regions = frames * p.wf.regions_per_frame;
    W.quorum = quorum;
    for (uint32_t q = 0u; q < 2u; q++) {
        if (q == 1u && p.same_sun != 0u) break;
        W.ray_o = p.wf.sun_o;
        W.ray_d = nullptr;
        W.ray_stop = p.wf.sun_stop;
        W.cursor = p.wf.cursors + q;
        W.kind = q;
        W.dir = q ? p.light.wi_reuse : p.light.wi;
        hipLaunchKernelGGL((k_wf_occl<true, 7>), dim3(sun_grid), block, 0, stream, W);
    }
    W.ray_o = p.wf.ibl_o;
    W.ray_d = p.wf.ibl_d;
    W.ray_stop = nullptr;
    W.cursor = p.wf.cursors + 2u;
    W.kind = 2u;
    hipLaunchKernelGGL((k_wf_occl<false, 8>), dim3(ibl_grid), block, 0, stream, W);
    return hipGetLastError();
}
hipError_t launch_trace_init(const FrameParams &p, hipStream_t stream) {
    if (frame_grid(p) == 0u) return hipSuccess;
    hipLaunchKernelGGL(k_trace_init, dim3(frame_grid(p)), dim3(kWave), 0, stream, p);
    return hipGetLastError();
}
hipError_t launch_merge(const FrameParams &p, hipStream_t stream) {
    if (frame_grid(p) == 0u) return hipSuccess;
    hipLaunchKernelGGL(k_merge, dim3(frame_grid(p)), dim3(kWave), 0, stream, p);
    return hipGetLastError();
// ... 40 lines not shown
hipError_t launch_drape_pack(const DrapePackParams &p, hipStream_t stream) {
    if (p.rows == 0u || p.cols == 0u) return hipSuccess;
    hipLaunchKernelGGL(k_drape_pack, dim3((p.cols + 255u) / 256u, p.rows), dim3(256), 0, stream, p);
    return hipGetLastError();
}
hipError_t launch_ray_batch(const RayBatchParams &p, hipStream_t stream) {
    hipLaunchKernelGGL(k_ray_batch, dim3((p.n + kWave - 1) / kWave), dim3(kWave), 0, stream, p);
    return hipGetLastError();
}
hipError_t launch_query(const QueryParams &p, hipStream_t stream) {
    if (p.count == 0u) return hipSuccess;
    const dim3 grid((p.count + kWave - 1u) / kWave), block(kWave);
    with_mesh(has_mesh(p.frame), [&](auto M) { hipLaunchKernelGGL((k_query<M()>), grid, block, 0, stream, p); });
    return hipGetLastError();
}
hipError_t launch_raster(const RasterParams &p, hipStream_t stream) {
    const uint32_t total = p.rows * p.cols;
    if (total == 0u || p.target_count == 0u) return hipSuccess;
    const dim3 grid((total + kWave - 1u) / kWave), block(kWave);
    with_mesh(has_mesh(p.frame), [&](auto M) { hipLaunchKernelGGL((k_raster<M()>), grid, block, 0, stream, p); });
    return hipGetLastError();
}
hipError_t launch_horizon(const HorizonParams &p, hipStream_t stream) {
    const uint32_t total = p.rows * p.cols;
    if (total == 0u || p.azimuth_count == 0u) return hipSuccess;
    const uint32_t waves = p.block ? ((p.cols + 7u) >> 3) * ((p.rows + 7u) >> 3) : (total + kWave - 1u) / kWave;
    hipLaunchKernelGGL(k_horizon, dim3(waves), dim3(kWave), 0, stream, p);
    return hipGetLastError();
}
hipError_t launch_irradiation(const IrradiationParams &p, hipStream_t stream) {
    const uint32_t total = p.rows * p.cols;
    if (total == 0u) return hipSuccess;
    const dim3 grid((total + kWave - 1u) / kWave), block(kWave);
    with_mesh(has_mesh(p.frame), [&](auto M) { hipLaunchKernelGGL((k_irradiation<M()>), grid, block, 0, stream, p); });
    return hipGetLastError();
}
hipError_t launch_clearance(const ClearanceParams &p, hipStream_t stream) {
    const uint32_t total = p.rows * p.cols;
    if (total == 0u || p.observer_count == 0u) return hipSuccess;
    const uint32_t waves = p.block ? ((p.cols + 7u) >> 3) * ((p.rows + 7u) >> 3) : (total + kWave - 1u) / kWave;
    hipLaunchKernelGGL(k_clearance, dim3(waves), dim3(kWave), 0, stream, p);
    return hipGetLastError();
}
hipError_t launch_leaf_build(const PyramidBuildParams &p, hipStream_t stream) {
    dim3 block(16, 16), grid((p.leaf_dim_x + 15) / 16, (p.leaf_dim_y + 15) / 16);
    hipLaunchKernelGGL(k_leaf_build, grid, block, 0, stream, p);
    return hipGetLastError();
}
hipError_t launch_band_build(const BandBuildParams &p, hipStream_t stream) {
    dim3 block(16, 16), grid((p.width + 15) / 16, (p.height + 15) / 16);
    hipLaunchKernelGGL(k_band_build, grid, block, 0, stream, p);
    return hipGetLastError();
}
hipError_t launch_level_build(const LevelBuildParams &p, hipStream_t stream) {
    dim3 block(16, 16), grid((p.dst_dim_x + 15) / 16, (p.dst_dim_y + 15) / 16);
    hipLaunchKernelGGL(k_level_build, grid, block, 0, stream, p);
    return hipGetLastError();
}

}

#if defined(F3D_MESH_STATS)
extern "C" int f3d_debug_mesh_stats(unsigned long long *out, int reset) {
    if (reset) {
        unsigned long long zero[8] = {};
        return (int)hipMemcpyToSymbol(HIP_SYMBOL(f3d::g_mesh_stats), zero, sizeof(zero));
    }
    return (int)hipMemcpyFromSymbol(out, HIP_SYMBOL(f3d::g_mesh_stats), 8 * sizeof(unsigned long long));
}
#endif
```

forge3d_amd/csrc/f3d_launch.h:

```cpp
#pragma once

#include <hip/hip_runtime.h>

#include "f3d_aether.h"
#include "f3d_build.h"
#include "f3d_drape.h"
#include "f3d_scene.h"

namespace f3d {

struct RayBatchParams {
    TerrainDev terrain;
    const float4 *rays;
    uint32_t n;
    uint32_t any_hit, apply_curvature;
    uint32_t start_in_cell;
    uint32_t *out_hit;
    float *out_t;
    float *out_normal;
};

struct ResolveParams {
    FrameParams frame;
    uint32_t frames;
    uint8_t *rgba;
    float *albedo, *normal;
    AetherDev aether;
    const float *depth;
};

hipError_t launch_head(const FrameParams &p, hipStream_t stream);
hipError_t launch_frame(const FrameParams &p, int variant, hipStream_t stream);
hipError_t launch_trace(const FrameParams &p, uint32_t frames, hipStream_t stream);
hipError_t launch_trace_wavefront(const FrameParams &p, uint32_t frames, uint32_t quorum, hipStream_t stream);
hipError_t launch_merge(const FrameParams &p, hipStream_t stream);
hipError_t launch_trace_init(const FrameParams &p, hipStream_t stream);
uint32_t frame_tile_count(const FrameParams &p, uint32_t *grid);
hipError_t launch_tile_order(const FrameParams &p, const uint32_t *cost, uint32_t *order, hipStream_t stream);
hipError_t launch_gbuffer(const FrameParams &p, float4 *gbuffer_n, float *depth, hipStream_t stream);
hipError_t launch_sky_blocks(const FrameParams &p, uint32_t *blocks, bool enabled, hipStream_t stream);
uint32_t sky_block_count(const FrameParams &p);
hipError_t launch_rearm(const RearmParams &p, hipStream_t stream);
hipError_t launch_reaim(const RearmParams &p, hipStream_t stream);
hipError_t launch_resolve(const ResolveParams &p, hipStream_t stream);
hipError_t launch_drape_pack(const DrapePackParams &p, hipStream_t stream);
hipError_t launch_ray_batch(const RayBatchParams &p, hipStream_t stream);
hipError_t launch_query(const QueryParams &p, hipStream_t stream);
hipError_t launch_raster(const RasterParams &p, hipStream_t stream);
hipError_t launch_horizon(const HorizonParams &p, hipStream_t stream);
hipError_t launch_irradiation(const IrradiationParams &p, hipStream_t stream);
hipError_t launch_clearance(const ClearanceParams &p, hipStream_t stream);
hipError_t launch_leaf_build(const PyramidBuildParams &p, hipStream_t stream);
hipError_t launch_level_build(const LevelBuildParams &p, hipStream_t stream);
hipError_t launch_band_build(const BandBuildParams &p, hipStream_t stream);
void horizon_table_dims(uint32_t cell_w, uint32_t cell_h, uint32_t *level, uint32_t *bx, uint32_t *bz);
hipError_t launch_horizon_build(const TerrainDev &terrain, float *table, hipStream_t stream);

}
```

forge3d_amd/csrc/f3d_lds.h:

```cpp
#pragma once

#include "f3d_march.h"

namespace f3d {

constexpr int kWave = 64;

__device__ __forceinline__ uint32_t lane_now() {
    uint32_t l;
    asm volatile("v_mbcnt_lo_u32_b32 %0, -1, 0\n\tv_mbcnt_hi_u32_b32 %0, -1, %0" : "=v"(l));
    return l;
}

constexpr int kParkRow = kFifoWords * kLeafFifoRows, kParkHead = 6, kParkWords = 8;
constexpr int kBoardRow = kParkRow + kParkHead + 1;
constexpr uint32_t kBoardBit = 0x80000000u;
constexpr int kLdsRows = kParkRow + kParkWords > kMaxLevels ? kParkRow + kParkWords : kMaxLevels;
constexpr int kLdsWords = kLdsRows * kWave + 4 * kMaxLevels;
template <int BOARD_ROW, bool MESH_STACK = true, bool SHARE_CLOSEST = false>
struct LdsPendingAt {
    static constexpr bool kShareClosest = SHARE_CLOSEST;
    static constexpr bool kMesh = MESH_STACK;
    uint32_t *col;
    const uint32_t *table;
// ... 65 lines not shown
                               __ATOMIC_RELAXED, __HIP_MEMORY_SCOPE_WAVEFRONT);
    }
    __device__ __forceinline__ uint32_t nearest_get(uint32_t owner) const {
        const uint32_t w = board()[owner & (kWave - 1u)];
        return (w & kBoardBit) != 0u ? 0x07FFFFFFu - (w & 0x07FFFFFFu) : kNoNearest;
    }
    __device__ __forceinline__ unsigned long long ballot(bool pred) const { return __ballot(pred); }
    __device__ __forceinline__ float shfl(float v, int src) const { return __shfl(v, src, kWave); }
    __device__ __forceinline__ uint32_t shfl(uint32_t v, int src) const { return (uint32_t)__shfl((int)v, src, kWave); }
    __device__ __forceinline__ float fast_log2(float x) const { return __builtin_amdgcn_logf(x); }
    __device__ __forceinline__ float fast_exp2(float x) const { return __builtin_amdgcn_exp2f(x); }
    template <bool CURVED>
    __device__ __forceinline__ void deal(const TerrainDev &T, MarchSlice &s, MarchState &m) const {
        march_deal<CURVED>(T, s, m, *this);
    }
    __device__ __forceinline__ void band_entry(const TerrainDev &, uint32_t level, uint32_t &offset,
                                               uint32_t &shift) const {
        const uint2 e = *reinterpret_cast<const uint2 *>(table + 4u * level);
        offset = e.x;
        shift = e.y;
    }
    __device__ __forceinline__ void level_entry(const TerrainDev &, uint32_t level, uint32_t &offset,
                                                uint32_t &tiles_x) const {
        const uint2 e = *reinterpret_cast<const uint2 *>(table + 4u * level + 2u);
        offset = e.x;
        tiles_x = e.y;
    }
};
using LdsPending = LdsPendingAt<kBoardRow>;
#ifndef F3D_WF_PARK
#define F3D_WF_PARK 8
#endif
constexpr int kPathParkRows = F3D_WF_PARK;
constexpr int kPathParkRow0 = kParkRow + 1;
constexpr int kCompactRows = kParkRow + 1 + kPathParkRows;
constexpr int kCompactLdsWords = kCompactRows * kWave + 4 * kMaxLevels;
#if !defined(F3D_WF_NO_SHARE_CLOSEST)
using LdsPendingCompact = LdsPendingAt<kParkRow, false, true>;
#else
using LdsPendingCompact = LdsPendingAt<kParkRow, false, false>;
#endif
struct LdsPendingTerrainOnly : LdsPending {
    static constexpr bool kMesh = false;
};
template <bool MESH>
struct PendingFor {
    using type = LdsPending;
};
template <>
struct PendingFor<false> {
    using type = LdsPendingTerrainOnly;
};

template <class Pending = LdsPending>
__device__ __forceinline__ Pending make_pending(uint32_t *lds, const TerrainDev &T, uint32_t rows = kLdsRows) {
    const uint32_t lane = threadIdx.x & (kWave - 1u);
    if (lane < kMaxLevels) {
        uint32_t *e = lds + rows * kWave + 4 * lane;
        e[0] = T.band_offset[lane];
        e[1] = T.band_shift[lane];
        e[2] = T.node_offset[lane];
        e[3] = T.tiles_x[lane];
    }
    __syncthreads();
    return Pending{lds + lane, lds + rows * kWave, T.leaf_quorum ? T.leaf_quorum : kDefaultLeafQuorum,
                   T.share_below ? (T.share_below < 64u ? T.share_below : 64u) : kShareBelow};
}

}
```

forge3d_amd/csrc/f3d_march.h:

```cpp
#pragma once

#include "f3d_trace.h"

namespace f3d {

template <bool CURVED>
F3D_HD float march_height(const RayCtx &r, float t) {
    const float lin = f_fma(t, r.d.y, r.o.y);
    return CURVED ? f_fma(t * t, r.c2, lin) : lin;
}

template <bool CURVED>
F3D_HD bool march_band_rejects(const RayCtx &r, float t0, float t1, float mn, float mx) {
#if !defined(F3D_PACKED_F32)
    const float y0 = march_height<CURVED>(r, t0), y1 = march_height<CURVED>(r, t1);
#else
    const F2 tt = f2(t0, t1);
    F2 yy = fma2(tt, f2(r.d.y, r.d.y), f2(r.o.y, r.o.y));
    if (CURVED) yy = fma2(tt * tt, f2(r.c2, r.c2), yy);
    const float y0 = yy.x, y1 = yy.y;
#endif
    float lo = f_min(y0, y1);
    if (CURVED) {
        if (r.has_vertex && r.vertex >= t0 && r.vertex <= t1) lo = f_min(lo, march_height<true>(r, r.vertex));
    }
    return (lo > mx) | (f_max(y0, y1) < mn);
}

#ifndef F3D_LEAF_FIFO
#define F3D_LEAF_FIFO 4
#endif
constexpr uint32_t kLeafFifo = F3D_LEAF_FIFO;
constexpr uint32_t kLeafFifoRows = kLeafFifo + 1u;
#ifndef F3D_FIFO_WORDS
#define F3D_FIFO_WORDS 3
#endif
constexpr uint32_t kFifoWords = F3D_FIFO_WORDS;
static_assert(kFifoWords == 1u || kFifoWords == 3u, "F3D_FIFO_WORDS: 1 (cell only) or 3 (cell, lo, hi)");
#ifndef F3D_STEPS_PER_VOTE
#define F3D_STEPS_PER_VOTE 8
#endif
constexpr uint32_t kStepsPerVote = F3D_STEPS_PER_VOTE;
#ifndef F3D_STEPS_PER_VOTE_SHARED
#define F3D_STEPS_PER_VOTE_SHARED 4
#endif
constexpr uint32_t kStepsPerVoteShared = F3D_STEPS_PER_VOTE_SHARED;
constexpr uint32_t kTieFlag = 0x80000000u, kTieSecond = 0x40000000u, kTieZFwd = 0x20000000u, kTieXFwd = 0x10000000u;
F3D_HD uint32_t tie_entry(uint32_t X, uint32_t Z, bool x_forward, bool z_forward) {
    return kTieFlag | (z_forward ? kTieZFwd : 0u) | (x_forward ? kTieXFwd : 0u) | (Z << 14) | X;
}

struct MarchState {
    float t_cur;
    uint32_t level, nx, nz;
    bool marching, unverified_start;
#if !defined(F3D_NO_BAND_PREFETCH)
    float band_mn, band_mx;
    float mesh_mn, mesh_mx;
#endif
};

constexpr uint32_t kMeshCell = 0x4000u, kMeshOnly = 0x8000u;
template <bool FUSE = false, class Ctx>
F3D_HD void march_fetch(const TerrainDev &T, MarchState &m, Ctx &ctx) {
#if !defined(F3D_NO_BAND_PREFETCH)
    uint32_t band_offset, band_shift;
    ctx.band_entry(T, m.level, band_offset, band_shift);
    const NodeRec band = T.bands[band_offset + (m.nz << band_shift) + m.nx];
    m.band_mn = band.mn;
    m.band_mx = band.mx;
    if (FUSE) {
        const NodeRec mesh = T.mesh_bands[band_offset + (m.nz << band_shift) + m.nx];
        m.mesh_mn = mesh.mn;
        m.mesh_mx = mesh.mx;
    }
#else
    static_assert(!FUSE, "the fused mesh band rides with the band prefetch");
#endif
}

F3D_HD void march_root_interval(const TerrainDev &T, const RayCtx &r, float &lo, float &hi) {
    const float ax = (plane_at(T.origin_x, 0u, T.spacing_x) - r.o.x) * r.inv_x;
    const float bx = (plane_at(T.origin_x, T.cell_w, T.spacing_x) - r.o.x) * r.inv_x;
    const float az = (plane_at(T.origin_z, 0u, T.spacing_z) - r.o.z) * r.inv_z;
    const float bz = (plane_at(T.origin_z, T.cell_h, T.spacing_z) - r.o.z) * r.inv_z;
    lo = f_max(f_max(f_min(ax, bx), f_min(az, bz)), r.tmin);
    hi = f_min(f_min(f_max(ax, bx), f_max(az, bz)), r.tmax);
}

F3D_HD MarchState march_begin(const TerrainDev &T, const RayCtx &r, bool start_in_cell) {
    MarchState m;
    float hi;
    march_root_interval(T, r, m.t_cur, hi);
    m.marching = !(m.t_cur > hi);
    m.level = T.mip_count - 1u;
    m.nx = 0u;
    m.nz = 0u;
    m.unverified_start = false;
    if (start_in_cell && !(m.t_cur > r.tmin)) {
        const float fx = f_floor((f_fma(m.t_cur, r.d.x, r.o.x) - T.origin_x) * T.inv_spacing_x);
        const float fz = f_floor((f_fma(m.t_cur, r.d.z, r.o.z) - T.origin_z) * T.inv_spacing_z);
        m.nx = sat_u32(fx);
        m.nz = sat_u32(fz);
        m.nx = m.nx < T.cell_w - 1u ? m.nx : T.cell_w - 1u;
        m.nz = m.nz < T.cell_h - 1u ? m.nz : T.cell_h - 1u;
        m.level = 0u;
        m.unverified_start = true;
    }
    return m;
}

template <bool CURVED, bool SLICED, bool VERIFY = true, bool FUSE = false, class Ctx>
F3D_HD void march_step(const TerrainDev &T, const RayCtx &r, MarchState &m, uint32_t &queued, Ctx &ctx, bool any_hit,
                       float t_stop = 3.0e38f) {
    ctx.note(0);
    const uint32_t top = T.mip_count - 1u;
    const uint32_t level = m.level, nx = m.nx, nz = m.nz;
    const bool x_forward = !(r.d.x < 0.0f), z_forward = !(r.d.z < 0.0f);
    const uint32_t cx0 = nx << level, cz0 = nz << level;
    uint32_t cx1 = (nx + 1u) << level, cz1 = (nz + 1u) << level;
    cx1 = cx1 < T.cell_w ? cx1 : T.cell_w;
    cz1 = cz1 < T.cell_h ? cz1 : T.cell_h;
#if !defined(F3D_PACKED_F32)
    const float tx0 = (plane_at(T.origin_x, cx0, T.spacing_x) - r.o.x) * r.inv_x;
    const float tx1 = (plane_at(T.origin_x, cx1, T.spacing_x) - r.o.x) * r.inv_x;
    const float tz0 = (plane_at(T.origin_z, cz0, T.spacing_z) - r.o.z) * r.inv_z;
    const float tz1 = (plane_at(T.origin_z, cz1, T.spacing_z) - r.o.z) * r.inv_z;
#else
    const F2 grid_o = f2(T.origin_x, T.origin_z), grid_s = f2(T.spacing_x, T.spacing_z);
    const F2 ray_o = f2(r.o.x, r.o.z), ray_inv = f2(r.inv_x, r.inv_z);
    const F2 t_lo = (fma2(f2((float)cx0, (float)cz0), grid_s, grid_o) - ray_o) * ray_inv;
    const F2 t_hi = (fma2(f2((float)cx1, (float)cz1), grid_s, grid_o) - ray_o) * ray_inv;
    const float tx0 = t_lo.x, tz0 = t_lo.y, tx1 = t_hi.x, tz1 = t_hi.y;
#endif
    const float x_out = f_max(tx0, tx1), z_out = f_max(tz0, tz1);
    const float enter = f_max(f_min(tx0, tx1), f_min(tz0, tz1)), exit = f_min(x_out, z_out);
    if (VERIFY && m.unverified_start && !(enter <= m.t_cur && m.t_cur <= exit)) {
        m.level = top;
        m.nx = 0u;
        m.nz = 0u;
    } else {
        const float lo = f_max(enter, r.tmin), hi = f_min(exit, r.tmax);
#if !defined(F3D_NO_BAND_PREFETCH)
        const NodeRec band{m.band_mn, m.band_mx};
#else
        uint32_t band_offset, band_shift;
        ctx.band_entry(T, level, band_offset, band_shift);
        const NodeRec band = T.bands[band_offset + (nz << band_shift) + nx];
#endif
        const bool terrain_pass = !(lo > hi) & !march_band_rejects<CURVED>(r, lo, hi, band.mn, band.mx);
        const bool mesh_pass = FUSE ? (!(lo > hi) & !march_band_rejects<false>(r, lo, hi, m.mesh_mn, m.mesh_mx)) : false;
        const bool pass = terrain_pass | mesh_pass;
        if (pass) ctx.note(-1);
#if defined(F3D_BRANCHLESS_STEP)
        {
            static_assert(!FUSE, "the branch-free A/B form of the step has no fused mesh band");
            const bool down = pass & (level > 0u), leaf = pass & (level == 0u);
            const uint32_t cl = level > 0u ? level - 1u : 0u;
            const uint32_t xm = (2u * nx + 1u) << cl, zm = (2u * nz + 1u) << cl;
            const float txm = (plane_at(T.origin_x, xm, T.spacing_x) - r.o.x) * r.inv_x;
            const float tzm = (plane_at(T.origin_z, zm, T.spacing_z) - r.o.z) * r.inv_z;
            uint32_t ix = (x_forward != (txm <= m.t_cur)) ? 0u : 1u;
            uint32_t iz = (z_forward != (tzm <= m.t_cur)) ? 0u : 1u;
            ix = xm < T.cell_w ? ix : 0u;
            iz = zm < T.cell_h ? iz : 0u;
#if !defined(F3D_NO_CORNER_TIES)
            if (any_hit && down && (txm == m.t_cur || tzm == m.t_cur)) {
                uint32_t lv = level;
                F3D_OPAQUE(lv);
                const uint32_t ex1 = (nx + 1u) << lv, ez1 = (nz + 1u) << lv;
                const uint32_t xin = x_forward ? nx << lv : (ex1 < T.cell_w ? ex1 : T.cell_w);
                const uint32_t zin = z_forward ? nz << lv : (ez1 < T.cell_h ? ez1 : T.cell_h);
                const float txin = (plane_at(T.origin_x, xin, T.spacing_x) - r.o.x) * r.inv_x;
                const float tzin = (plane_at(T.origin_z, zin, T.spacing_z) - r.o.z) * r.inv_z;
                if (txm == m.t_cur && tzin == m.t_cur && xm < T.cell_w) {
                    ctx.fifo_put(queued, tie_entry(xm, zin, x_forward, z_forward), m.t_cur, m.t_cur);
                    queued++;
                } else if (tzm == m.t_cur && txin == m.t_cur && zm < T.cell_h) {
                    ctx.fifo_put(queued, tie_entry(xin, zm, x_forward, z_forward), m.t_cur, m.t_cur);
                    queued++;
                }
            }
#endif
            if (leaf) ctx.note(1);
            ctx.fifo_put(queued, nx | (nz << 16), lo, hi);
            queued += leaf ? 1u : 0u;
            const bool cross_x = x_out <= z_out, cross_z = z_out <= x_out;
#if !defined(F3D_NO_CORNER_TIES)
            if (any_hit && !down && cross_x && cross_z && exit < r.tmax) {
                uint32_t lv = level;
                F3D_OPAQUE(lv);
                const uint32_t ex1 = (nx + 1u) << lv, ez1 = (nz + 1u) << lv;
                const uint32_t X = x_forward ? (ex1 < T.cell_w ? ex1 : T.cell_w) : nx << lv;
                const uint32_t Z = z_forward ? (ez1 < T.cell_h ? ez1 : T.cell_h) : nz << lv;
                ctx.fifo_put(queued, tie_entry(X, Z, x_forward, z_forward), exit, exit);
                queued++;
            }
#endif
            const uint32_t qx = nx + ((cross_x && x_forward) ? 1u : 0u) - ((cross_x && !x_forward) ? 1u : 0u);
            const uint32_t qz = nz + ((cross_z && z_forward) ? 1u : 0u) - ((cross_z && !z_forward) ? 1u : 0u);
            const bool left = !(exit < r.tmax) | (SLICED & !(exit < t_stop)) | ((qx << level) >= T.cell_w) |
                              ((qz << level) >= T.cell_h) | (march_height<CURVED && !FUSE>(r, exit) > r.y_exit);
            const bool up = level < top && (((qx ^ nx) | (qz ^ nz)) > 1u);
            m.nx = down ? 2u * nx + ix : (up ? qx >> 1 : qx);
            m.nz = down ? 2u * nz + iz : (up ? qz >> 1 : qz);
// ... 515 lines not shown
```

forge3d_amd/csrc/f3d_scene.h:

```cpp
#pragma once

#include "f3d_math.h"

namespace f3d {

constexpr uint32_t kMaxLevels = 16;
constexpr uint32_t kRestirMCap = 512;
constexpr uint32_t kWelfordWindow = 32;
constexpr uint32_t kHaloRows = 4;
#if !defined(F3D_SPATIAL_REACH_HI)
#define F3D_SPATIAL_REACH_HI 4
#endif
constexpr uint32_t kSpatialReachLo = 3, kSpatialReachHi = F3D_SPATIAL_REACH_HI;
static_assert(kHaloRows >= kSpatialReachHi && kHaloRows >= kSpatialReachLo, "a strip's halo covers the spatial pass");
constexpr uint32_t kIblSectors = 8;
constexpr uint32_t kDefaultLeafQuorum = 64;

struct alignas(16) LeafRec {
    float h00, h10, h01, h11;
};
struct alignas(8) NodeRec {
    float mn, mx;
};

F3D_HD uint32_t child_group_index(uint32_t px, uint32_t py, uint32_t tiles_x) {
    uint32_t tile = mul24((py >> 2), tiles_x) + (px >> 2);
    uint32_t g = (px & 1u) | ((py & 1u) << 1) | ((px & 2u) << 1) | ((py & 2u) << 2);
    return (tile << 6) | (g << 2);
}
F3D_HD uint32_t tiled_index(uint32_t x, uint32_t y, uint32_t tiles_x) {
    return child_group_index(x >> 1, y >> 1, tiles_x) | (x & 1u) | ((y & 1u) << 1);
}

struct TerrainDev {
    const LeafRec *leaves;
    const NodeRec *nodes;
    uint32_t node_offset[kMaxLevels];
    uint32_t tiles_x[kMaxLevels];
    const NodeRec *bands;
    uint32_t band_offset[kMaxLevels];
    uint32_t band_shift[kMaxLevels];
    uint32_t mip_count;
    uint32_t cell_w, cell_h;
    float origin_x, origin_z, spacing_x, spacing_z, inv_spacing_x, inv_spacing_z;
    float inv_two_r_prime;
    uint32_t curvature_enabled;
    const float *horizon;
    uint32_t horizon_level, horizon_bx;
    uint32_t leaf_quorum;
    uint32_t share_below;
    const NodeRec *mesh_bands;
    const uint32_t *mesh_cell_start;
    const float4 *mesh_cell_tris;
    float mesh_top;
    uint32_t mesh_reserved;
};

struct BvhNode {
    float bmin[3];
    uint32_t skip;
    float bmax[3];
    uint32_t leaf;
};
static_assert(sizeof(BvhNode) == 32, "BvhNode is two dwordx4 loads");

struct alignas(128) Bvh4Node {
    float lo_x[4], hi_x[4], lo_y[4], hi_y[4], lo_z[4], hi_z[4];
    uint32_t leaf[4];
    uint32_t first_child, inner, pad0, pad1;
};
static_assert(sizeof(Bvh4Node) == 128, "Bvh4Node is eight dwordx4 loads, one cache line");
constexpr uint32_t kBvh4MaxLevels = 15;

struct MeshDev {
    const float4 *vertices;
    const uint32_t *indices;
    uint32_t vertex_count, index_count;
    uint32_t traversal_mode;
    const BvhNode *bvh_nodes;
    const float4 *bvh_tris;
    uint32_t bvh_node_count;
    const Bvh4Node *bvh4_nodes;
    uint32_t bvh4_node_count;
};

struct EnvDev {
    const float4 *texels;
    uint32_t width, height;
    float intensity;
};

struct CameraDev {
    V3 origin, right, up, forward;
    float half_w, half_h;
    float exposure;
    uint32_t width, height;
    uint32_t seed_hi, seed_lo;
    float cone_delta;
};

F3D_HD float pixel_cone_delta_of(float half_w, float half_h, uint32_t width, uint32_t height) {
    const float px = half_w / (float)width, py = half_h / (float)height;
    const float plane = f_sqrt(px * px + py * py);
    return plane < 0.25f ? 1.01f * plane * (1.0f + plane * plane) : -1.0f;
}

struct LightDev {
    V3 wi;
// ... 150 lines not shown
```

forge3d_amd/csrc/f3d_setup.h:

```cpp
#pragma once

#include <chrono>
#include <cmath>
#include <cstdarg>
#include <cstdio>
#include <cstdlib>
#include <cstring>
#include <string>
#include <vector>

#include "../../include/f3d_terrain_pt.h"
#include "f3d_build.h"
#include "f3d_bvh.h"
#include "f3d_scene.h"

namespace f3d {

struct Failure {
    int status;
    std::string message;
};

[[noreturn]] inline void fail(int status, const char *fmt, ...) {
    char buf[1024];
// ... 219 lines not shown
        t.dim_y[l] = l == 0 ? pad8(t.cell_h) : pad8(lh);
        t.tiles_x[l] = t.dim_x[l] / 8u;
        if (l >= 1) {
            t.node_offset[l] = (uint32_t)t.node_count;
            t.node_count += (uint64_t)t.dim_x[l] * t.dim_y[l];
        }
        t.levels++;
        if (lw == 1 && lh == 1) break;
        lw = lw / 2 > 1 ? lw / 2 : 1;
        lh = lh / 2 > 1 ? lh / 2 : 1;
    }
    t.leaf_count = (uint64_t)t.dim_x[0] * t.dim_y[0];
    for (uint32_t l = 0; l < t.levels; l++) {
        uint32_t shift = 0;
        while ((1u << shift) < t.level_w[l]) shift++;
        uint32_t rows = (t.cell_h + (1u << l) - 1u) >> l;
        rows = rows < 1u ? 1u : (rows < t.level_h[l] ? rows : t.level_h[l]);
        t.band_offset[l] = (uint32_t)t.band_count;
        t.band_shift[l] = shift;
        t.band_rows[l] = rows;
        t.band_count += (uint64_t)t.level_w[l] * rows;
    }
    return t;
}

inline void apply_layout(const TableLayout &t, TerrainDev &dev) {
    for (uint32_t l = 0; l < kMaxLevels; l++) {
        dev.node_offset[l] = t.node_offset[l];
        dev.tiles_x[l] = t.tiles_x[l];
        dev.band_offset[l] = t.band_offset[l];
        dev.band_shift[l] = t.band_shift[l];
    }
    dev.mip_count = t.levels;
    dev.cell_w = t.cell_w;
    dev.cell_h = t.cell_h;
}

inline BandBuildParams band_build_params(const TableLayout &t, uint32_t l, const LeafRec *leaves, const NodeRec *nodes,
                                         NodeRec *bands) {
    BandBuildParams b{};
    b.leaves = leaves;
    b.src = l >= 1 ? nodes + t.node_offset[l] : nullptr;
    b.dst = bands + t.band_offset[l];
    b.level = l;
    b.width = t.level_w[l];
    b.height = t.band_rows[l];
    b.shift = t.band_shift[l];
    b.src_tiles_x = t.tiles_x[l];
    b.cell_w = t.cell_w;
    b.cell_h = t.cell_h;
    return b;
}

inline PyramidBuildParams leaf_build_params(const TableLayout &t, const float *heights, uint32_t w, uint32_t h,
                                            float exaggeration, LeafRec *leaves) {
    PyramidBuildParams b{};
    b.heights = heights;
    b.w = w;
    b.h = h;
    b.exaggeration = exaggeration;
    b.leaves = leaves;
    b.leaf_tiles_x = t.tiles_x[0];
    b.leaf_dim_x = t.dim_x[0];
    b.leaf_dim_y = t.dim_y[0];
    return b;
}

inline LevelBuildParams level_build_params(const TableLayout &t, uint32_t l, const LeafRec *leaves, NodeRec *nodes) {
    LevelBuildParams b{};
    b.leaves = leaves;
    b.src = l >= 2 ? nodes + t.node_offset[l - 1] : nullptr;
    b.dst = nodes + t.node_offset[l];
    b.level = l;
    b.src_w = t.level_w[l - 1];
    b.src_h = t.level_h[l - 1];
    b.dst_w = t.level_w[l];
    b.dst_h = t.level_h[l];
    b.src_tiles_x = t.tiles_x[l - 1];
    b.dst_tiles_x = t.tiles_x[l];
    b.dst_dim_x = t.dim_x[l];
    b.dst_dim_y = t.dim_y[l];
    b.cell_w = t.cell_w;
    b.cell_h = t.cell_h;
    return b;
}

inline bool fill_uniforms(const f3d_terrain_ref_desc &d, FrameParams &P) {
    const float kScaleMax = 65504.0f;
    const float exposure = f_clamp(d.exposure, 0.0f, kScaleMax);
    const float sun_intensity = f_clamp(d.sun_intensity, 0.0f, kScaleMax);
    const float sun_color[3] = {f_clamp(d.sun_color[0], 0.0f, kScaleMax), f_clamp(d.sun_color[1], 0.0f, kScaleMax),
                                f_clamp(d.sun_color[2], 0.0f, kScaleMax)};
    const float env_intensity = f_clamp(d.env_intensity, 0.0f, kScaleMax);

    if (!std::isfinite(d.observer_latitude_deg) || d.observer_latitude_deg < -90.0 || d.observer_latitude_deg > 90.0 ||
        !std::isfinite(d.observer_longitude_deg) || d.observer_longitude_deg < -180.0 ||
        d.observer_longitude_deg > 180.0)
        fail(F3D_STATUS_RENDER, "ray-origin latitude/longitude must be finite and in [-90,90]/[-180,180]");
    const double radius = effective_radius(d.earth_model, d.observer_latitude_deg, d.sphere_radius_m, d.refraction_model,
                                           d.pressure_mbar, d.temperature_c, d.refraction_k, (double)d.sun_azimuth_deg);
    const bool curved = std::isfinite(radius);

    P.terrain.origin_x = -0.5f * ((float)d.dem_width - 1.0f) * d.spacing_x;
    P.terrain.origin_z = -0.5f * ((float)d.dem_height - 1.0f) * d.spacing_z;
    P.terrain.spacing_x = d.spacing_x;
    P.terrain.spacing_z = d.spacing_z;
// ... 62 lines not shown
```

forge3d_amd/session.py:

```python
from __future__ import annotations

import ctypes as C

import numpy as np

from . import _native

HALO_ROWS = 4
RESERVOIR_BYTES = 16
WELFORD_WINDOW = 32


class TerrainSession:
    def __init__(self, heightmap, width, height, camera=None, *, row_begin=0, row_end=0, device=-1, stream=0,
                 memory_budget_bytes=0, kernel_variant=0, ext_reservoirs=(None, None), ext_stats=None, bands=0,
                 band_streams=0, mesh_builder=0, frames_in_flight=0,
                 spacing=(1.0, 1.0), exaggeration=1.0, albedo=(0.6, 0.6, 0.6), sun_azimuth_deg=315.0,
                 sun_elevation_deg=45.0, sun_intensity=2.5, sun_color=(1.0, 0.97, 0.92), env_map=None,
                 env_intensity=0.35, mesh_vertices=None, mesh_indices=None, spp=1, max_frames=512, min_frames=32,
                 variance_threshold=1e-3, seed=7, observer_latitude_deg=0.0, observer_longitude_deg=0.0,
                 earth_model="ellipsoid", sphere_radius_m=6_371_008.8, refraction_model="bennett",
                 refraction_k=0.13, pressure_mbar=1013.25, temperature_c=15.0, atmosphere=None):
        self._lib = _native.lib()
        self._handle = C.c_void_p(None)
# ... 654 lines not shown
            q.directions = terms.data_ptr() if k else None
            ptr = lambda t: None if t is None else t.data_ptr()
        else:
            if not wait:
                raise ValueError("wait=False is for tensor irradiations: results in host memory are there when the call returns")
            e_out = np.zeros((rows, cols), np.float32) if energy else None
            c_out = np.zeros((rows, cols), np.uint32) if count else None
            n_out = np.zeros((rows, cols, 3), np.float32) if normal else None
            q.directions = terms.ctypes.data if k else None
            ptr = lambda a: None if a is None else a.ctypes.data
        q.energy, q.count, q.normal = ptr(e_out), ptr(c_out), ptr(n_out)
        self._check(self._lib.f3d_session_irradiation(self._handle, C.byref(q), self._err, len(self._err)))
        return e_out, c_out, n_out

    def irradiation(self, directions, weights=None, *, horizontal: bool = False, curved: bool = True, terrain_only: bool = False,
                    lift: float = SURFACE_BIAS, region=None, count: bool = False, wait: bool = True):
        terms = self.irradiation_terms(directions, weights)
        flags = ((_native.IRRADIATION_HORIZONTAL if horizontal else 0) | (_native.IRRADIATION_CURVED if curved else 0)
                 | (_native.IRRADIATION_TERRAIN_ONLY if terrain_only else 0))
        e, c, _ = self._irradiation(terms, flags, lift, region, True, count, False, wait)
        return (e, c) if count else e

    def surface_normals(self, region=None, wait: bool = True):
        device = None
        if not wait:
            import torch

            device = torch.device("cuda", self._device if self._device >= 0 else torch.cuda.current_device())
        return self._irradiation(None, 0, 0.0, region, False, False, True, wait, device)[2]

    def insolation(self, track, *, dni=None, dhi=None, azimuths=16, **irradiation_kwargs) -> dict:
        from . import insolation as _insolation

        unknown = set(irradiation_kwargs) - {"horizontal", "curved", "terrain_only", "lift", "region"}
        if unknown:
            raise TypeError(f"insolation() got unexpected keyword arguments {sorted(unknown)}")
        hours = np.asarray(track["hours"], np.float64)
        if dni is None or dhi is None:
            clear = _insolation.clear_sky(track["elevation_deg"])
            dni = clear[0] if dni is None else dni
            dhi = clear[1] if dhi is None else dhi
        dni, dhi = np.asarray(dni, np.float64), np.asarray(dhi, np.float64)
        direct = self.irradiation(np.asarray(track["directions"], np.float32), (dni * hours).astype(np.float32), **irradiation_kwargs)
        sky = {k: v for k, v in irradiation_kwargs.items() if k in ("curved", "lift", "region")}
        diffuse = (self.sky_view_factor(azimuths, **sky) * np.float32((dhi * hours).sum())).astype(np.float32)
        return {"direct": direct, "diffuse": diffuse, "global": (direct + diffuse).astype(np.float32)}

    def certificates(self) -> dict:
        out = (C.c_uint64 * 2)()
        if self._lib.f3d_session_certificates(self._handle, out) != 0:
            raise RuntimeError("f3d_session_certificates failed")
        return {"sun_clear": int(out[0]), "primary_start": int(out[1])}

    def sky_blocks(self) -> dict:
        out = (C.c_uint32 * 4)()
        if self._lib.f3d_session_sky_blocks(self._handle, out) != 0:
            raise RuntimeError("f3d_session_sky_blocks failed")
        return {"blocks": int(out[0]), "deep_blocks": int(out[1]), "certified_pixels": int(out[2]), "deep_pixels": int(out[3])}

    def enqueue_frames(self, first_frame: int, count: int, collect_stats: bool = False):
        self._check(self._lib.f3d_session_enqueue_frames(self._handle, int(first_frame), int(count),
                                                         1 if collect_stats else 0, self._err, len(self._err)))

    def enqueue_trace(self, first_frame: int, count: int):
        self._check(self._lib.f3d_session_enqueue_trace(self._handle, int(first_frame), int(count), self._err, len(self._err)))

    def enqueue_merge(self, frame: int, collect_stats: bool = False):
        self._check(self._lib.f3d_session_enqueue_merge(self._handle, int(frame), 1 if collect_stats else 0, self._err, len(self._err)))

    def frames_in_flight(self) -> int:
        return int(self._lib.f3d_session_frames_in_flight(self._handle))

    def trace_batch(self, frame: int, remaining: int) -> int:
        return int(self._lib.f3d_session_trace_batch(self._handle, int(frame), int(remaining)))

    def retraced_pixels(self) -> int:
        total = C.c_uint64(0)
        self._lib.f3d_session_retraced_pixels(self._handle, C.byref(total))
        return int(total.value)

    FINGERPRINT_FIELDS = ("camera", "light", "terrain_scalars", "mesh_scalars", "scalars", "leaf_table", "band_tables",
                          "mesh_vertices", "mesh_indices", "bvh_nodes", "bvh_triangles", "environment", "gbuffer",
                          "reservoirs", "accumulation", "frame_heads", "drape")

    def fingerprint(self) -> dict:
        out = (C.c_uint64 * 17)()
        if self._lib.f3d_session_fingerprint(self._handle, out, 17) != 0:
            raise RuntimeError("f3d_session_fingerprint failed")
        return dict(zip(self.FINGERPRINT_FIELDS, (int(v) for v in out)))

    BVH_NODE = np.dtype([("bmin", "<f4", 3), ("skip", "<u4"), ("bmax", "<f4", 3), ("leaf", "<u4")])
    BVH4_NODE = np.dtype([("lo_x", "<f4", 4), ("hi_x", "<f4", 4), ("lo_y", "<f4", 4), ("hi_y", "<f4", 4), ("lo_z", "<f4", 4),
                          ("hi_z", "<f4", 4), ("leaf", "<u4", 4), ("first_child", "<u4"), ("inner", "<u4"), ("pad", "<u4", 2)])
    BVH_CORNER = np.dtype([("xyz", "<f4", 3), ("w", "<u4")])

    def mesh_tree(self):
        info = (C.c_uint32 * 4)()
        self._check(self._lib.f3d_session_mesh_tree(self._handle, info, None, 0, None, 0, self._err, len(self._err)))
        form, node_count, tri_count = int(info[0]), int(info[1]), int(info[2])
        nodes = np.zeros(node_count, self.BVH4_NODE if form == 2 else self.BVH_NODE)
        tris = np.zeros((tri_count, 3), self.BVH_CORNER)
        self._check(self._lib.f3d_session_mesh_tree(self._handle, info, nodes.ctypes.data, nodes.nbytes, tris.ctypes.data, tris.nbytes,
                                                    self._err, len(self._err)))
        if (int(info[0]), int(info[1]), int(info[2])) != (form, node_count, tri_count):
            raise RuntimeError("f3d_session_mesh_tree: the tree changed between the two calls")
        return form, nodes, tris
# ... 149 lines not shown
```

include/f3d_terrain_pt.h:

```cpp
#ifndef F3D_TERRAIN_PT_H
#define F3D_TERRAIN_PT_H

#include <stddef.h>
#include <stdint.h>

#ifdef __cplusplus
extern "C" {
#endif

#define F3D_ABI_VERSION 6u
#define F3D_STATUS_OK 0
#define F3D_STATUS_VALUE 1
#define F3D_STATUS_RENDER 2
#define F3D_STATUS_UPLOAD 3
#define F3D_STATUS_DEVICE 4

#define F3D_EARTH_FLAT 0
#define F3D_EARTH_SPHERE 1
#define F3D_EARTH_ELLIPSOID 2
#define F3D_REFRACTION_NONE 0
#define F3D_REFRACTION_BENNETT 1
#define F3D_REFRACTION_SAEMUNDSSON 2
#define F3D_REFRACTION_EFFECTIVE_RADIUS 3

// ... 83 lines not shown
int f3d_session_enqueue_merge(f3d_session *session, uint32_t frame, int32_t collect_stats, char *err, size_t errlen);
uint32_t f3d_session_frames_in_flight(f3d_session *session);
uint32_t f3d_session_trace_batch(f3d_session *session, uint32_t frame, uint32_t remaining);
int f3d_session_retraced_pixels(f3d_session *session, uint64_t *total);
int f3d_session_enqueue_frame_part(f3d_session *session, uint32_t frame, uint32_t part, int32_t collect_stats,
                                   char *err, size_t errlen);
int f3d_session_window_stats(f3d_session *session, float *max_m2, int32_t *nonfinite, char *err,
                             size_t errlen);
int f3d_session_halo(f3d_session *session, int32_t which, int32_t side, void **ptr, uint64_t *bytes);
typedef struct f3d_halo_stats {
    uint32_t reset;
    uint32_t frames_published;
    uint32_t timeouts, pulls;
    double wait_ms[2];
    double longest_wait_ms;
    double timeout_ms;
} f3d_halo_stats;
int f3d_session_halo_stats(f3d_session *session, f3d_halo_stats *out, char *err, size_t errlen);
typedef struct f3d_halo_export {
    uint8_t handle[3][64];
    uint64_t offset[3];
    uint64_t address[3];
    uint32_t rows, width;
    int32_t device;
    uint32_t pid;
} f3d_halo_export;
int f3d_session_halo_export(f3d_session *session, f3d_halo_export *out, char *err, size_t errlen);
int f3d_session_halo_connect(f3d_session *session, int32_t side, const f3d_halo_export *peer, char *err, size_t errlen);
int f3d_session_halo_probe(f3d_session *session, int32_t mode, uint32_t nonce, uint32_t *seen, char *err, size_t errlen);
int f3d_session_halo_status(f3d_session *session, uint32_t *timeouts, char *err, size_t errlen);
int f3d_session_enqueue_batch_strip(f3d_session *session, uint32_t first_frame, uint32_t count, int32_t collect_stats_on_last,
                                    char *err, size_t errlen);
int f3d_session_resolve(f3d_session *session, uint32_t frames, uint8_t *rgba, float *albedo,
                        float *normal, float *depth, int32_t *any_valid_reservoir, char *err,
                        size_t errlen);
int f3d_session_set_accumulation(f3d_session *session, const float *sums_rgba, char *err, size_t errlen);
int f3d_session_resolve_device(f3d_session *session, uint32_t frames, void *d_rgba, void *d_albedo,
                               void *d_normal, void *d_depth, char *err, size_t errlen);
#define F3D_SETUP_PHASES 8
int f3d_session_setup_ms(f3d_session *session, double *out, uint32_t count);
typedef struct f3d_session_rearm_desc {
    uint32_t struct_size;
    float sun_azimuth_deg, sun_elevation_deg, sun_intensity;
    float sun_color[3];
    float exposure, env_intensity;
    uint32_t seed, max_frames, min_frames;
    float variance_threshold;
    double observer_latitude_deg, observer_longitude_deg, pressure_mbar, temperature_c;
} f3d_session_rearm_desc;
int f3d_session_rearm(f3d_session *session, const f3d_session_rearm_desc *desc, char *err, size_t errlen);
int f3d_session_render(f3d_session *session, f3d_terrain_ref_out *out, char *err, size_t errlen);
int f3d_session_certificates(f3d_session *session, uint64_t out[2]);
int f3d_session_sky_blocks(f3d_session *session, uint32_t out[4]);
typedef struct f3d_session_reaim_desc {
    uint32_t struct_size;
    float cam_origin[3], cam_look_at[3], cam_up[3];
    float fov_y_deg;
    f3d_session_rearm_desc arm;
} f3d_session_reaim_desc;
int f3d_session_reaim(f3d_session *session, const f3d_session_reaim_desc *desc, char *err, size_t errlen);
typedef struct f3d_session_remesh_desc {
    uint32_t struct_size;
    const float *mesh_vertices;
    uint32_t mesh_vertex_count;
    const uint32_t *mesh_indices;
    uint32_t mesh_index_count;
    f3d_session_reaim_desc aim;
} f3d_session_remesh_desc;
int f3d_session_remesh(f3d_session *session, const f3d_session_remesh_desc *desc, char *err, size_t errlen);
typedef struct f3d_session_reterrain_desc {
    uint32_t struct_size;
    const float *heights;
    uint32_t width, height;
    uint32_t x0, y0;
    float exaggeration;
    f3d_session_reaim_desc aim;
} f3d_session_reterrain_desc;
int f3d_session_reterrain(f3d_session *session, const f3d_session_reterrain_desc *desc, char *err, size_t errlen);
#define F3D_QUERY_CLOSEST 0u
#define F3D_QUERY_OCCLUSION 1u
#define F3D_QUERY_PIXELS 2u
#define F3D_QUERY_TERRAIN_ONLY 1u
#define F3D_QUERY_CURVED 2u
#define F3D_QUERY_DEVICE_POINTERS 4u
#define F3D_QUERY_NO_WAIT 8u
#define F3D_QUERY_SCRATCH_BYTES_PER_RAY 80u
typedef struct f3d_session_query_desc {
    uint32_t struct_size;
    uint32_t mode;
    uint32_t flags;
    uint32_t count;
    const void *rays;
    uint32_t *kind;
    float *t;
    float *normal;
    float *position;
    uint32_t *primitive;
    float *direction;
} f3d_session_query_desc;
int f3d_session_query(f3d_session *session, const f3d_session_query_desc *desc, char *err, size_t errlen);
#define F3D_RASTER_TOWARD_POINT 0u
#define F3D_RASTER_ALONG_DIRECTION 1u
#define F3D_RASTER_TERRAIN_ONLY 1u
#define F3D_RASTER_CURVED 2u
#define F3D_RASTER_DEVICE_POINTERS 4u
#define F3D_RASTER_NO_WAIT 8u
// ... 187 lines not shown
    uint32_t layer_width, layer_height;
    int32_t offset_x, offset_y;
    const uint8_t *base;
    const uint8_t *layer;
    float base_alpha, layer_alpha;
    uint32_t max_alpha;
} f3d_composite_desc;
int f3d_smoke_composite(const f3d_composite_desc *desc, uint8_t *out_rgba, double *kernel_seconds, char *err, size_t errlen);

typedef struct f3d_smoke_seq f3d_smoke_seq;
typedef struct f3d_smoke_seq_stats_t {
    uint64_t scratch_bytes;
    uint32_t shadow_list_chunks;
    uint32_t shadow_list_chunks_used;
    uint32_t shadow_list_slots_per_chunk;
    uint32_t reserved;
} f3d_smoke_seq_stats_t;
int f3d_smoke_seq_create(void *stream_solver, void *stream_march, f3d_smoke_seq **out, char *err, size_t errlen);
void f3d_smoke_seq_destroy(f3d_smoke_seq *seq);
int f3d_smoke_seq_streams(f3d_smoke_seq *seq, void **stream_solver, void **stream_march);
int f3d_smoke_seq_step(f3d_smoke_seq *seq, f3d_smoke_state *state, const f3d_smoke_step_settings *settings, const f3d_smoke_emitter *emitters,
                       uint32_t emitter_count, uint32_t steps, double *device_seconds, char *err, size_t errlen);
int f3d_smoke_seq_render(f3d_smoke_seq *seq, const f3d_smoke_volume *volume, const f3d_smoke_view *view, const f3d_smoke_settings *settings,
                         uint8_t *rgba, double *kernel_seconds, char *err, size_t errlen);
int f3d_smoke_seq_composite(f3d_smoke_seq *seq, const f3d_composite_desc *desc, uint8_t *out_rgba, double *kernel_seconds, char *err, size_t errlen);
int f3d_smoke_seq_stats(f3d_smoke_seq *seq, f3d_smoke_seq_stats_t *out, char *err, size_t errlen);

typedef struct f3d_aether_ref_desc {
    uint32_t struct_size;
    uint32_t dem_width, dem_height;
    const float *heights;
    float spacing_x, spacing_z, exaggeration;
    float cam_origin[3], cam_look_at[3], cam_up[3], fov_y_deg;
    float sun_azimuth_deg, sun_elevation_deg, sun_intensity;
    float turbidity, ozone_du, mie_g, ground_albedo;
    uint32_t width, height, seed, spp;
    int32_t enabled;
    float variance_threshold;
} f3d_aether_ref_desc;
typedef struct f3d_aether_ref_out {
    float *mean_xyz;
    float *linear_rgb;
    float variance;
    int32_t converged;
    uint64_t terrain_primary_hits;
    uint64_t gpu_resource_bytes;
    double kernel_seconds;
} f3d_aether_ref_out;
int f3d_aether_reference_render(const f3d_aether_ref_desc *desc, f3d_aether_ref_out *out, char *err, size_t errlen);

int f3d_build_minmax_mips(const float *heights, uint32_t width, uint32_t height, float *levels_out,
                          uint32_t *dims_out, uint32_t max_levels, uint64_t *total_floats, char *err,
                          size_t errlen);
int f3d_terrain_trace_batch(const float *heights, uint32_t width, uint32_t height, float origin_x,
                            float origin_z, float spacing_x, float spacing_z, float exaggeration,
                            float inv_two_r_prime, uint32_t curvature_enabled, const float *rays,
                            uint32_t n, int32_t any_hit, int32_t apply_curvature, uint32_t *out_hit,
                            float *out_t, float *out_normal, char *err, size_t errlen);
int f3d_effective_radius_m(int32_t earth_model, double latitude_deg, double sphere_radius_m,
                           int32_t refraction_model, double pressure_mbar, double temperature_c,
                           double refraction_k, double azimuth_deg, double *radius_out, char *err,
                           size_t errlen);

void f3d_scene_cache_limit(uint32_t entries);
uint32_t f3d_scene_cache_entries(void);

int f3d_device_count(void);
const char *f3d_device_name(int32_t device);
const char *f3d_version(void);
uint32_t f3d_abi_version(void);
const char *f3d_source_digest(void);
void f3d_debug_poison(int32_t pattern);

#ifdef __cplusplus
}
#endif
#endif
```

Before: 9562.

## Add tilted-plane node slabs to cull terrain pyramid nodes during ray marching

Builds a per-node table of sloped bounding slabs (a plane fit plus lo/hi offsets) for each pyramid level above the leaves, using a parallel piecewise reduction with atomic min/max for large nodes. During the march, a node that passes the flat min/max band test is also tested against its slab, and skipped when the ray segment lies entirely above the tilted upper bound. The goal is to reject more nodes on sloped terrain and so cut descent steps. In exchange it adds a one-time setup build, extra memory traffic and registers for slab prefetch in the march loop, and new kernel variants that run without slabs.

```diff
diff --git a/forge3d_amd/_native.py b/forge3d_amd/_native.py
--- a/forge3d_amd/_native.py
+++ b/forge3d_amd/_native.py
@@ -257,6 +257,7 @@
     ("f3d_session_draped", C.c_int, [C.c_void_p, _P(C.c_uint32)]),
     ("f3d_session_certificates", C.c_int, [C.c_void_p, _P(C.c_uint64)]),
     ("f3d_session_sky_blocks", C.c_int, [C.c_void_p, _P(C.c_uint32)]),
+    ("f3d_session_node_slab_bytes", C.c_uint64, [C.c_void_p]),
     ("f3d_session_debug_wave_times", C.c_int, [C.c_void_p, C.c_void_p]),
     ("f3d_session_halo", C.c_int, [C.c_void_p, C.c_int32, C.c_int32, _P(C.c_void_p), _P(C.c_uint64)]),
     ("f3d_session_resolve", C.c_int, [C.c_void_p, C.c_uint32, C.c_void_p, C.c_void_p, C.c_void_p, C.c_void_p,
@@ -285,6 +286,8 @@
                                      C.c_float, C.c_float, C.c_float, C.c_float, C.c_void_p, C.c_char_p, C.c_size_t]),
     ("f3d_build_minmax_mips", C.c_int, [C.c_void_p, C.c_uint32, C.c_uint32, C.c_void_p, C.c_void_p, C.c_uint32,
                                         _P(C.c_uint64), C.c_char_p, C.c_size_t]),
+    ("f3d_build_node_slabs", C.c_int, [C.c_void_p, C.c_uint32, C.c_uint32, C.c_float, C.c_float, C.c_float, C.c_float, C.c_float,
+                                       C.c_void_p, C.c_uint64, _P(C.c_uint64), C.c_char_p, C.c_size_t]),
     ("f3d_terrain_trace_batch", C.c_int, [C.c_void_p, C.c_uint32, C.c_uint32, C.c_float, C.c_float, C.c_float,
                                           C.c_float, C.c_float, C.c_float, C.c_uint32, C.c_void_p, C.c_uint32,
                                           C.c_int32, C.c_int32, C.c_void_p, C.c_void_p, C.c_void_p, C.c_char_p,
diff --git a/forge3d_amd/csrc/f3d_build.h b/forge3d_amd/csrc/f3d_build.h
--- a/forge3d_amd/csrc/f3d_build.h
+++ b/forge3d_amd/csrc/f3d_build.h
@@ -33,6 +33,19 @@
     uint32_t shift;
     uint32_t src_tiles_x;
     uint32_t cell_w, cell_h;
+};
+
+struct SlabBuildParams {
+    const LeafRec *leaves;
+    uint32_t leaf_tiles_x;
+    const NodeRec *band;
+    SlabRec *dst;
+    uint32_t level;
+    uint32_t width, height;
+    uint32_t shift;
+    uint32_t cell_w, cell_h;
+    float spacing_x, spacing_z;
+    float reach_x, reach_z;
 };
 
 F3D_HD float min4(const LeafRec &h) { return f_min(f_min(f_min(h.h00, h.h10), h.h01), h.h11); }
@@ -75,6 +88,72 @@
     B.dst[tiled_index(x, y, B.dst_tiles_x)] = NodeRec{mn, mx};
 }
 
+constexpr float kSlabTau = 1.52587890625e-05f;
+constexpr float kSlabFar = 8.0f;
+F3D_HD float slab_reach(float origin, uint32_t cells, float spacing) {
+    const float width = (float)cells * f_abs(spacing);
+    return f_max(f_abs(origin), f_abs(f_fma((float)cells, spacing, origin))) + width;
+}
+F3D_HD void slab_attach(TerrainDev &T, const SlabRec *slabs) {
+    T.slabs = slabs;
+    T.slab_far_x = kSlabFar * slab_reach(T.origin_x, T.cell_w, T.spacing_x);
+    T.slab_far_z = kSlabFar * slab_reach(T.origin_z, T.cell_h, T.spacing_z);
+}
+F3D_HD bool slab_extent(const SlabBuildParams &B, uint32_t x, uint32_t z, uint32_t &cx0, uint32_t &cz0, uint32_t &cx1, uint32_t &cz1) {
+    cx0 = x << B.level;
+    cz0 = z << B.level;
+    cx1 = (x + 1u) << B.level;
+    cz1 = (z + 1u) << B.level;
+    cx1 = cx1 < B.cell_w ? cx1 : B.cell_w;
+    cz1 = cz1 < B.cell_h ? cz1 : B.cell_h;
+    return cx0 < B.cell_w && cz0 < B.cell_h;
+}
+F3D_HD float slab_sample(const SlabBuildParams &B, uint32_t i, uint32_t j) {
+    const uint32_t cx = i < B.cell_w ? i : B.cell_w - 1u, cz = j < B.cell_h ? j : B.cell_h - 1u;
+    const LeafRec h = B.leaves[tiled_index(cx, cz, B.leaf_tiles_x)];
+    return i > cx ? (j > cz ? h.h11 : h.h10) : (j > cz ? h.h01 : h.h00);
+}
+F3D_HD void slab_slopes(const SlabBuildParams &B, uint32_t cx0, uint32_t cz0, uint32_t cx1, uint32_t cz1, float &a, float &b) {
+    const float h00 = slab_sample(B, cx0, cz0), h10 = slab_sample(B, cx1, cz0);
+    const float h01 = slab_sample(B, cx0, cz1), h11 = slab_sample(B, cx1, cz1);
+    a = ((h10 + h11) - (h00 + h01)) / (2.0f * ((float)(cx1 - cx0) * B.spacing_x));
+    b = ((h01 + h11) - (h00 + h10)) / (2.0f * ((float)(cz1 - cz0) * B.spacing_z));
+    if (!(f_abs(a) < 1e6f)) a = 0.0f;
+    if (!(f_abs(b) < 1e6f)) b = 0.0f;
+}
+F3D_HD float slab_term(const SlabBuildParams &B, float a, float b, uint32_t cx0, uint32_t cz0, uint32_t i, uint32_t j, float h) {
+    const float dx = (float)(i - cx0) * B.spacing_x, dz = (float)(j - cz0) * B.spacing_z;
+    return f_fma(-b, dz, f_fma(-a, dx, h));
+}
+F3D_HD SlabRec slab_finish(const SlabBuildParams &B, uint32_t x, uint32_t z, float a, float b, float lo, float hi) {
+    const NodeRec band = B.band[((size_t)z << B.shift) + x];
+    const float h_abs = f_max(f_abs(band.mn), f_abs(band.mx));
+    const float margin = kSlabTau * f_fma(f_abs(b), B.reach_z, f_fma(f_abs(a), B.reach_x, h_abs));
+    SlabRec rec{a, b, (lo + 0.0f) - margin, (hi + 0.0f) + margin};
+    if (!(rec.lo <= rec.hi)) rec = SlabRec{0.0f, 0.0f, -__builtin_inff(), __builtin_inff()};
+    return rec;
+}
+F3D_HD void slab_cell_terms(const SlabBuildParams &B, float a, float b, uint32_t cx0, uint32_t cz0, uint32_t cx, uint32_t cz, float &lo, float &hi) {
+    const LeafRec h = B.leaves[tiled_index(cx, cz, B.leaf_tiles_x)];
+    const float g00 = slab_term(B, a, b, cx0, cz0, cx, cz, h.h00), g10 = slab_term(B, a, b, cx0, cz0, cx + 1u, cz, h.h10);
+    const float g01 = slab_term(B, a, b, cx0, cz0, cx, cz + 1u, h.h01), g11 = slab_term(B, a, b, cx0, cz0, cx + 1u, cz + 1u, h.h11);
+    lo = f_min(lo, f_min(f_min(g00, g10), f_min(g01, g11)));
+    hi = f_max(hi, f_max(f_max(g00, g10), f_max(g01, g11)));
+}
+F3D_HD void slab_build_at(const SlabBuildParams &B, uint32_t x, uint32_t z) {
+    SlabRec rec{0.0f, 0.0f, -__builtin_inff(), __builtin_inff()};
+    uint32_t cx0, cz0, cx1, cz1;
+    if (slab_extent(B, x, z, cx0, cz0, cx1, cz1)) {
+        float a, b;
+        slab_slopes(B, cx0, cz0, cx1, cz1, a, b);
+        float lo = __builtin_inff(), hi = -__builtin_inff();
+        for (uint32_t cz = cz0; cz < cz1; cz++)
+            for (uint32_t cx = cx0; cx < cx1; cx++) slab_cell_terms(B, a, b, cx0, cz0, cx, cz, lo, hi);
+        rec = slab_finish(B, x, z, a, b, lo, hi);
+    }
+    B.dst[((size_t)z << B.shift) + x] = rec;
+}
+
 F3D_HD void band_build_at(const BandBuildParams &B, uint32_t x, uint32_t z) {
     NodeRec out{__builtin_inff(), -__builtin_inff()};
     if (B.level == 0u) {
diff --git a/forge3d_amd/csrc/f3d_frame.h b/forge3d_amd/csrc/f3d_frame.h
--- a/forge3d_amd/csrc/f3d_frame.h
+++ b/forge3d_amd/csrc/f3d_frame.h
@@ -458,17 +458,26 @@
     frame_in_batch = group % gridDim.y;
     slot = (group / gridDim.y) * kNumXcd + xcd;
 }
-template <int MIN_WAVES, uint32_t S, bool MESH = false>
-__global__ __launch_bounds__(kWave, MIN_WAVES) void k_trace(const FrameParams P) {
-    __shared__ __attribute__((aligned(16))) uint32_t lds[kLdsWords];
+template <uint32_t S, bool MESH, bool SLAB>
+__device__ __forceinline__ void trace_wave(const FrameParams &P, uint32_t *lds) {
     const unsigned long long t_start = wall_clock64();
-    typename PendingFor<MESH>::type pend{make_pending(lds, P.terrain)};
+    typename FramePendingFor<MESH, SLAB>::type pend{make_pending(lds, P.terrain)};
     uint32_t gx = 0u, gy = 0u, tile, frame_in_batch, slot;
     batch_slot(frame_in_batch, slot);
     const bool active = tile_pixel<S>(P, gx, gy, tile, P.tile_order, slot);
     trace_lanes<S>(P, P.frame_index + frame_in_batch, tile, active, pend);
     if (lane_now() == 0u && frame_in_batch == 0u && P.tile_cost && tile != 0xFFFFFFFFu)
         P.tile_cost[tile] = (uint32_t)(wall_clock64() - t_start);
+}
+template <int MIN_WAVES, uint32_t S, bool MESH = false>
+__global__ __launch_bounds__(kWave, MIN_WAVES) void k_trace(const FrameParams P) {
+    __shared__ __attribute__((aligned(16))) uint32_t lds[kLdsWords];
+    trace_wave<S, MESH, true>(P, lds);
+}
+template <int MIN_WAVES, uint32_t S, bool MESH = false>
+__global__ __launch_bounds__(kWave, MIN_WAVES) void k_trace_bands(const FrameParams P) {
+    __shared__ __attribute__((aligned(16))) uint32_t lds[kLdsWords];
+    trace_wave<S, MESH, false>(P, lds);
 }
 
 __global__ __launch_bounds__(kWave) void k_merge(const FrameParams P) {
@@ -491,7 +500,7 @@
         }
     }
     if (__ballot(redo) != 0ull) {
-        LdsPending pend = make_pending(lds, P.terrain);
+        WithSlabs<LdsPending> pend{make_pending(lds, P.terrain)};
         if (redo) {
             m2 = fix_pixel(P, gx, gy, rec, pixels, pend);
             atomicAdd(&P.fix_count[2], 1u);
@@ -555,7 +564,7 @@
     if (active) P.head[(size_t)(gy - P.row_begin) * P.cam.width + gx] = pack_head(frame_head<true>(P, gx, gy));
 }
 
-template <uint32_t S, bool MESH, bool DRAPE>
+template <uint32_t S, bool MESH, bool DRAPE, bool SLAB = true>
 __device__ __forceinline__ void frame_wave(const FrameParams &P, uint32_t *lds) {
     const unsigned long long t_start = wall_clock64();
     uint32_t gx = 0u, gy = 0u, tile;
@@ -567,7 +576,7 @@
             if ((P.sky_blocks[block] & kSkyBlockDeep) != 0u) return;
         }
     }
-    typename PendingFor<MESH>::type pend{make_pending(lds, P.terrain)};
+    typename FramePendingFor<MESH, SLAB>::type pend{make_pending(lds, P.terrain)};
     float m2 = 0.0f;
     if constexpr (S == 1u) {
         if (active) m2 = frame_pixel<DRAPE>(P, gx, gy, pend);
@@ -592,10 +601,20 @@
     __shared__ __attribute__((aligned(16))) uint32_t lds[kLdsWords];
     frame_wave<S, MESH, false>(P, lds);
 }
+template <int VARIANT, int MIN_WAVES = 1, uint32_t S = 1u, bool MESH = false>
+__global__ __launch_bounds__(kWave, MIN_WAVES) void k_frame_bands(const FrameParams P) {
+    __shared__ __attribute__((aligned(16))) uint32_t lds[kLdsWords];
+    frame_wave<S, MESH, false, false>(P, lds);
+}
 template <int MIN_WAVES, uint32_t S, bool MESH>
 __global__ __launch_bounds__(kWave, MIN_WAVES) void k_frame_drape(const FrameParams P) {
     __shared__ __attribute__((aligned(16))) uint32_t lds[kLdsWords];
     frame_wave<S, MESH, true>(P, lds);
+}
+template <int MIN_WAVES, uint32_t S, bool MESH>
+__global__ __launch_bounds__(kWave, MIN_WAVES) void k_frame_drape_bands(const FrameParams P) {
+    __shared__ __attribute__((aligned(16))) uint32_t lds[kLdsWords];
+    frame_wave<S, MESH, true, false>(P, lds);
 }
 
 struct SkyBlocksParams {
@@ -682,7 +701,8 @@
     const RayCtx r = make_ray(B.terrain, V3{a.x, a.y, a.z}, a.w, V3{b.x, b.y, b.z}, b.w, B.apply_curvature != 0u);
     TraceHit h;
     if (B.any_hit >= 2u) {
-        h = march_ray(B.terrain, r, B.any_hit == 2u, B.start_in_cell != 0u, pend);
+        WithSlabs<LdsPending> slabbed{pend};
+        h = march_ray(B.terrain, r, B.any_hit == 2u, B.start_in_cell != 0u, slabbed);
     } else {
         h = trace_terrain(B.terrain, r, B.any_hit != 0u, pend);
     }
@@ -838,6 +858,70 @@
     if (x < B.dst_dim_x && y < B.dst_dim_y) level_build_at(B, x, y);
 }
 
+constexpr uint32_t kSlabSerialLevel = 3u, kSlabPieceShift = 6u, kSlabPiece = 1u << kSlabPieceShift, kSlabThreads = 256u;
+__device__ __forceinline__ uint32_t slab_ordered(float f) {
+    const uint32_t b = f_bits(f);
+    return (b & 0x80000000u) ? ~b : b | 0x80000000u;
+}
+__device__ __forceinline__ float slab_unordered(uint32_t u) { return f_from_bits((u & 0x80000000u) ? u & 0x7FFFFFFFu : ~u); }
+__global__ __launch_bounds__(256) void k_slab_serial(const SlabBuildParams B) {
+    const uint32_t x = blockIdx.x * 16u + (threadIdx.x & 15u), z = blockIdx.y * 16u + (threadIdx.x >> 4);
+    if (x < B.width && z < B.height) slab_build_at(B, x, z);
+}
+__global__ __launch_bounds__(256) void k_slab_begin(const SlabBuildParams B) {
+    const uint32_t x = blockIdx.x * 16u + (threadIdx.x & 15u), z = blockIdx.y * 16u + (threadIdx.x >> 4);
+    if (x >= B.width || z >= B.height) return;
+    uint32_t cx0, cz0, cx1, cz1;
+    float a = 0.0f, b = 0.0f;
+    if (slab_extent(B, x, z, cx0, cz0, cx1, cz1)) slab_slopes(B, cx0, cz0, cx1, cz1, a, b);
+    B.dst[((size_t)z << B.shift) + x] = SlabRec{a, b, f_from_bits(slab_ordered(__builtin_inff())), f_from_bits(slab_ordered(-__builtin_inff()))};
+}
+__global__ __launch_bounds__(kSlabThreads) void k_slab_pieces(const SlabBuildParams B) {
+    __shared__ float part_lo[kSlabThreads / kWave], part_hi[kSlabThreads / kWave];
+    const uint32_t x = blockIdx.x & (B.width - 1u), z = blockIdx.x >> B.shift;
+    uint32_t cx0, cz0, cx1, cz1;
+    if (z >= B.height || !slab_extent(B, x, z, cx0, cz0, cx1, cz1)) return;
+    const uint32_t up = B.level > kSlabPieceShift ? B.level - kSlabPieceShift : 0u, across = 1u << up;
+    const uint32_t px0 = cx0 + (blockIdx.y & (across - 1u)) * kSlabPiece, pz0 = cz0 + (blockIdx.y >> up) * kSlabPiece;
+    if (px0 >= cx1 || pz0 >= cz1) return;
+    const uint32_t px1 = px0 + kSlabPiece < cx1 ? px0 + kSlabPiece : cx1, pz1 = pz0 + kSlabPiece < cz1 ? pz0 + kSlabPiece : cz1;
+    SlabRec *rec = B.dst + (((size_t)z << B.shift) + x);
+    const float a = rec->a, b = rec->b;
+    float lo = __builtin_inff(), hi = -__builtin_inff();
+    const uint32_t w = px1 - px0, n = w * (pz1 - pz0);
+    for (uint32_t k = threadIdx.x; k < n; k += kSlabThreads) slab_cell_terms(B, a, b, cx0, cz0, px0 + k % w, pz0 + k / w, lo, hi);
+#pragma unroll
+    for (int d = kWave / 2; d >= 1; d >>= 1) {
+        lo = f_min(lo, __shfl_xor(lo, d, kWave));
+        hi = f_max(hi, __shfl_xor(hi, d, kWave));
+    }
+    if ((threadIdx.x & (kWave - 1u)) == 0u) {
+        part_lo[threadIdx.x / kWave] = lo;
+        part_hi[threadIdx.x / kWave] = hi;
+    }
+    __syncthreads();
+    if (threadIdx.x == 0u) {
+        for (uint32_t i = 1u; i < kSlabThreads / kWave; i++) {
+            lo = f_min(lo, part_lo[i]);
+            hi = f_max(hi, part_hi[i]);
+        }
+        atomicMin(reinterpret_cast<uint32_t *>(&rec->lo), slab_ordered(lo));
+        atomicMax(reinterpret_cast<uint32_t *>(&rec->hi), slab_ordered(hi));
+    }
+}
+__global__ __launch_bounds__(256) void k_slab_end(const SlabBuildParams B) {
+    const uint32_t x = blockIdx.x * 16u + (threadIdx.x & 15u), z = blockIdx.y * 16u + (threadIdx.x >> 4);
+    if (x >= B.width || z >= B.height) return;
+    SlabRec *rec = B.dst + (((size_t)z << B.shift) + x);
+    uint32_t cx0, cz0, cx1, cz1;
+    if (!slab_extent(B, x, z, cx0, cz0, cx1, cz1)) {
+        *rec = SlabRec{0.0f, 0.0f, -__builtin_inff(), __builtin_inff()};
+        return;
+    }
+    const SlabRec r = *rec;
+    *rec = slab_finish(B, x, z, r.a, r.b, slab_unordered(f_bits(r.lo)), slab_unordered(f_bits(r.hi)));
+}
+
 struct HorizonBuildParams {
     TerrainDev terrain;
     uint32_t level, bx, bz;
diff --git a/forge3d_amd/csrc/f3d_host.hip b/forge3d_amd/csrc/f3d_host.hip
--- a/forge3d_amd/csrc/f3d_host.hip
+++ b/forge3d_amd/csrc/f3d_host.hip
@@ -98,6 +98,7 @@
         }
     } own_mesh;
     uint64_t scene_counted = 0;
+    uint64_t slab_bytes = 0;
     struct OwnTerrain {
         LeafRec *leaves = nullptr;
         NodeRec *bands = nullptr;
@@ -577,6 +578,33 @@
         hip_check(launch_trace_init(P, s.stream), "trace prediction init");
     }
     clock.lap(kSetupPasses);
+
+    if (const char *off = getenv("F3D_NODE_SLABS"); slab_buildable(s.tables.layout) && !(off && off[0] == '0')) {
+        std::lock_guard<std::mutex> lock(g_scene_mutex);
+        const TerrainDev &T = P.terrain;
+        const size_t bytes = (size_t)slab_count(s.tables.layout) * sizeof(SlabRec);
+        const CachedTables::Slabs *have = nullptr;
+        for (const auto &sl : s.scene->slabs)
+            if (sl.origin_x == T.origin_x && sl.origin_z == T.origin_z && sl.spacing_x == T.spacing_x && sl.spacing_z == T.spacing_z) have = &sl;
+        const bool room = s.mem.device_bytes + bytes <= s.budget;
+        if (!have && room && s.scene->slabs.size() < kMaxSlabPlacements) {
+            try {
+                CachedTables::Slabs sl{T.origin_x, T.origin_z, T.spacing_x, T.spacing_z, nullptr, bytes};
+                sl.table = build_slabs(s.scene->slab_mem, s.tables.layout, T, s.tables.leaves, s.tables.bands, s.stream);
+                hip_check(hipStreamSynchronize(s.stream), "node slab build");
+                s.scene->slabs.push_back(sl);
+                have = &s.scene->slabs.back();
+                clock.lap(kSetupTables);
+            } catch (const Failure &) {
+                (void)hipGetLastError();
+                have = nullptr;
+            }
+        }
+        if (have && room) {
+            slab_attach(P.terrain, have->table);
+            s.slab_bytes = have->bytes;
+        }
+    }
 }
 
 template <class Launch>
@@ -1107,6 +1135,8 @@
         t.mesh_bands = nullptr;
         t.mesh_cell_start = nullptr;
         t.mesh_cell_tris = nullptr;
+        t.slabs = nullptr;
+        t.slab_far_x = t.slab_far_z = 0.0f;
         MeshDev m = P.mesh;
         m.vertices = nullptr;
         m.indices = nullptr;
@@ -1205,6 +1235,8 @@
         return F3D_STATUS_DEVICE;
     }
 }
+
+uint64_t f3d_session_node_slab_bytes(const f3d_session *s) { return s ? s->slab_bytes : 0u; }
 
 int f3d_session_sky_blocks(f3d_session *s, uint32_t out[4]) {
     if (!s || !out) return F3D_STATUS_VALUE;
@@ -1342,6 +1374,43 @@
     return rc;
 }
 
+int f3d_build_node_slabs(const float *heights, uint32_t width, uint32_t height, float origin_x, float origin_z, float spacing_x,
+                         float spacing_z, float exaggeration, float *records_out, uint64_t capacity, uint64_t *count, char *err,
+                         size_t errlen) {
+    if (err && errlen) err[0] = 0;
+    Ledger mem;
+    int rc = F3D_STATUS_OK;
+    try {
+        if (width < 2 || height < 2)
+            fail(F3D_STATUS_UPLOAD, "terrain heightfield must be at least 2x2 texels, got %ux%u", width, height);
+        int ndev = 0;
+        if (hipGetDeviceCount(&ndev) != hipSuccess || ndev <= 0)
+            fail(F3D_STATUS_DEVICE, "no HIP device available: libf3dhip has no CPU fallback");
+        const TableLayout L = table_layout(width, height);
+        const uint64_t records = slab_count(L);
+        if (count) *count = records;
+        if (records_out && records != 0u) {
+            if (capacity < records) fail(F3D_STATUS_VALUE, "node slab table holds %llu records, the buffer %llu", (unsigned long long)records, (unsigned long long)capacity);
+            const size_t dem_n = (size_t)width * height;
+            float *d_h = (float *)mem.alloc(dem_n * sizeof(float), "DEM upload");
+            hip_check(hipMemcpy(d_h, heights, dem_n * sizeof(float), hipMemcpyHostToDevice), "DEM upload");
+            TerrainTables t = build_tables(mem, d_h, width, height, exaggeration, nullptr, true);
+            TerrainDev placed = t.dev;
+            placed.origin_x = origin_x;
+            placed.origin_z = origin_z;
+            placed.spacing_x = spacing_x;
+            placed.spacing_z = spacing_z;
+            const SlabRec *slabs = build_slabs(mem, L, placed, t.leaves, t.bands, nullptr);
+            hip_check(hipDeviceSynchronize(), "node slab build");
+            hip_check(hipMemcpy(records_out, slabs, (size_t)records * sizeof(SlabRec), hipMemcpyDeviceToHost), "readback");
+        }
+    } catch (const Failure &f) {
+        rc = report(f, err, errlen);
+    }
+    mem.release();
+    return rc;
+}
+
 int f3d_terrain_trace_batch(const float *heights, uint32_t width, uint32_t height, float origin_x, float origin_z,
                             float spacing_x, float spacing_z, float exaggeration, float inv_two_r_prime,
                             uint32_t curvature_enabled, const float *rays, uint32_t n, int32_t any_hit,
@@ -1370,6 +1439,7 @@
         B.terrain.inv_spacing_z = 1.0f / spacing_z;
         B.terrain.inv_two_r_prime = inv_two_r_prime;
         B.terrain.curvature_enabled = curvature_enabled;
+        if (((uint32_t)any_hit & 2u) != 0u && slab_buildable(t.layout)) slab_attach(B.terrain, build_slabs(mem, t.layout, B.terrain, t.leaves, t.bands, nullptr));
         float4 *d_rays = (float4 *)mem.alloc((size_t)n * 32, "rays");
         hip_check(hipMemcpy(d_rays, rays, (size_t)n * 32, hipMemcpyHostToDevice), "ray upload");
         B.rays = d_rays;
diff --git a/forge3d_amd/csrc/f3d_host_mem.h b/forge3d_amd/csrc/f3d_host_mem.h
--- a/forge3d_amd/csrc/f3d_host_mem.h
+++ b/forge3d_amd/csrc/f3d_host_mem.h
@@ -192,6 +192,14 @@
     return t;
 }
 
+constexpr size_t kMaxSlabPlacements = 4;
+SlabRec *build_slabs(Ledger &mem, const TableLayout &L, const TerrainDev &placed, const LeafRec *leaves, const NodeRec *bands, hipStream_t stream) {
+    SlabRec *slabs = (SlabRec *)mem.alloc((size_t)slab_count(L) * sizeof(SlabRec), "node slabs");
+    for (uint32_t l = 1; l < L.levels; l++)
+        hip_check(launch_slab_build(slab_build_params(L, l, placed, leaves, bands, slabs), stream), "node slab build");
+    return slabs;
+}
+
 }
 
 enum SetupPhase { kSetupTotal = 0, kSetupValidate, kSetupHash, kSetupUpload, kSetupTables, kSetupScene, kSetupAlloc, kSetupPasses, kSetupPhases };
@@ -224,10 +232,18 @@
         uint32_t level, bx, bz;
     };
     std::vector<Horizon> horizons;
+    struct Slabs {
+        float origin_x, origin_z, spacing_x, spacing_z;
+        SlabRec *table;
+        size_t bytes;
+    };
+    std::vector<Slabs> slabs;
+    Ledger slab_mem;
     ~CachedTables() {
         int prev = -1;
         (void)hipGetDevice(&prev);
         (void)hipSetDevice(device);
+        slab_mem.release();
         mem.release();
         if (prev >= 0) (void)hipSetDevice(prev);
     }
diff --git a/forge3d_amd/csrc/f3d_host_update.h b/forge3d_amd/csrc/f3d_host_update.h
--- a/forge3d_amd/csrc/f3d_host_update.h
+++ b/forge3d_amd/csrc/f3d_host_update.h
@@ -99,7 +99,12 @@
     }
 };
 
-void check_budget(const f3d_session &s, uint64_t planned, const char *update, const char *brings) {
+void drop_slabs(f3d_session &s) {
+    s.params.terrain.slabs = nullptr;
+    s.slab_bytes = 0u;
+}
+void check_budget(f3d_session &s, uint64_t planned, const char *update, const char *brings) {
+    if (planned <= s.budget && planned + s.slab_bytes > s.budget) drop_slabs(s);
     if (planned > s.budget)
         fail(F3D_STATUS_RENDER, "%s exceeds the memory budget: %s the tracked total to %llu > limit %llu", update, brings,
              (unsigned long long)planned, (unsigned long long)s.budget);
@@ -283,6 +288,7 @@
         }
         O = N;
     }
+    drop_slabs(s);
     join_bands(s);
     if (!O.live) {
         hip_check(hipMemcpyAsync(O.leaves, s.tables.leaves, leaf_bytes, hipMemcpyDeviceToDevice, s.stream), "re-terrain copy");
diff --git a/forge3d_amd/csrc/f3d_kernels.hip b/forge3d_amd/csrc/f3d_kernels.hip
--- a/forge3d_amd/csrc/f3d_kernels.hip
+++ b/forge3d_amd/csrc/f3d_kernels.hip
@@ -58,7 +58,23 @@
     const bool mesh = has_mesh(p) || force_mesh;
     const int budget = variant % 1000;
     bool known = false;
-    if (p.drape) {
+    if (p.terrain.slabs == nullptr) {
+        if (p.drape) {
+            known = budget == 0 && with_lanes(lanes, [&](auto S) {
+                with_mesh(mesh, [&](auto M) { hipLaunchKernelGGL((k_frame_drape_bands<kDrapeWaves, S(), M()>), grid, block, 0, stream, p); });
+            });
+        } else if (budget == 0) {
+            known = with_lanes(lanes, [&](auto S) {
+                with_mesh(mesh, [&](auto M) { hipLaunchKernelGGL((k_frame_bands<0, 6, S(), M()>), grid, block, 0, stream, p); });
+            });
+        } else if (budget == 104 && lanes == 1u) {
+            known = true;
+            with_mesh(mesh, [&](auto M) { hipLaunchKernelGGL((k_frame_bands<0, 4, 1u, M()>), grid, block, 0, stream, p); });
+        } else if (budget == 105 && lanes == 4u) {
+            known = true;
+            with_mesh(mesh, [&](auto M) { hipLaunchKernelGGL((k_frame_bands<0, 5, 4u, M()>), grid, block, 0, stream, p); });
+        }
+    } else if (p.drape) {
         known = budget == 0 && with_lanes(lanes, [&](auto S) {
             with_mesh(mesh, [&](auto M) { hipLaunchKernelGGL((k_frame_drape<kDrapeWaves, S(), M()>), grid, block, 0, stream, p); });
         });
@@ -80,7 +96,10 @@
     if (frame_grid(p, lanes) == 0u || frames == 0u) return hipSuccess;
     const dim3 grid(frame_grid(p, lanes), frames), block(kWave);
     const bool known = with_lanes(lanes, [&](auto S) {
-        with_mesh(has_mesh(p), [&](auto M) { hipLaunchKernelGGL((k_trace<6, S(), M()>), grid, block, 0, stream, p); });
+        with_mesh(has_mesh(p), [&](auto M) {
+            if (p.terrain.slabs == nullptr) hipLaunchKernelGGL((k_trace_bands<6, S(), M()>), grid, block, 0, stream, p);
+            else hipLaunchKernelGGL((k_trace<6, S(), M()>), grid, block, 0, stream, p);
+        });
     });
     return known ? hipGetLastError() : hipErrorInvalidValue;
 }
@@ -227,6 +246,19 @@
     hipLaunchKernelGGL(k_band_build, grid, block, 0, stream, p);
     return hipGetLastError();
 }
+hipError_t launch_slab_build(const SlabBuildParams &p, hipStream_t stream) {
+    const dim3 block(256), nodes((p.width + 15) / 16, (p.height + 15) / 16);
+    if (p.level <= kSlabSerialLevel) {
+        hipLaunchKernelGGL(k_slab_serial, nodes, block, 0, stream, p);
+        return hipGetLastError();
+    }
+    const uint32_t up = p.level > kSlabPieceShift ? p.level - kSlabPieceShift : 0u;
+    if (up > 7u) return hipErrorInvalidValue;
+    hipLaunchKernelGGL(k_slab_begin, nodes, block, 0, stream, p);
+    hipLaunchKernelGGL(k_slab_pieces, dim3(p.width * p.height, 1u << (2u * up)), dim3(kSlabThreads), 0, stream, p);
+    hipLaunchKernelGGL(k_slab_end, nodes, block, 0, stream, p);
+    return hipGetLastError();
+}
 hipError_t launch_level_build(const LevelBuildParams &p, hipStream_t stream) {
     dim3 block(16, 16), grid((p.dst_dim_x + 15) / 16, (p.dst_dim_y + 15) / 16);
     hipLaunchKernelGGL(k_level_build, grid, block, 0, stream, p);
diff --git a/forge3d_amd/csrc/f3d_launch.h b/forge3d_amd/csrc/f3d_launch.h
--- a/forge3d_amd/csrc/f3d_launch.h
+++ b/forge3d_amd/csrc/f3d_launch.h
@@ -53,6 +53,7 @@
 hipError_t launch_leaf_build(const PyramidBuildParams &p, hipStream_t stream);
 hipError_t launch_level_build(const LevelBuildParams &p, hipStream_t stream);
 hipError_t launch_band_build(const BandBuildParams &p, hipStream_t stream);
+hipError_t launch_slab_build(const SlabBuildParams &p, hipStream_t stream);
 void horizon_table_dims(uint32_t cell_w, uint32_t cell_h, uint32_t *level, uint32_t *bx, uint32_t *bz);
 hipError_t launch_horizon_build(const TerrainDev &terrain, float *table, hipStream_t stream);
 
diff --git a/forge3d_amd/csrc/f3d_lds.h b/forge3d_amd/csrc/f3d_lds.h
--- a/forge3d_amd/csrc/f3d_lds.h
+++ b/forge3d_amd/csrc/f3d_lds.h
@@ -141,6 +141,20 @@
     using type = LdsPendingTerrainOnly;
 };
 
+template <class Base>
+struct WithSlabs : Base {
+    static constexpr bool kSlab = true;
+    __device__ __forceinline__ explicit WithSlabs(const LdsPending &p) : Base{p} {}
+};
+template <bool MESH, bool SLAB = true>
+struct FramePendingFor {
+    using type = WithSlabs<typename PendingFor<MESH>::type>;
+};
+template <bool MESH>
+struct FramePendingFor<MESH, false> {
+    using type = typename PendingFor<MESH>::type;
+};
+
 template <class Pending = LdsPending>
 __device__ __forceinline__ Pending make_pending(uint32_t *lds, const TerrainDev &T, uint32_t rows = kLdsRows) {
     const uint32_t lane = threadIdx.x & (kWave - 1u);
diff --git a/forge3d_amd/csrc/f3d_march.h b/forge3d_amd/csrc/f3d_march.h
--- a/forge3d_amd/csrc/f3d_march.h
+++ b/forge3d_amd/csrc/f3d_march.h
@@ -25,6 +25,21 @@
         if (r.has_vertex && r.vertex >= t0 && r.vertex <= t1) lo = f_min(lo, march_height<true>(r, r.vertex));
     }
     return (lo > mx) | (f_max(y0, y1) < mn);
+}
+
+template <class Ctx, class = void>
+struct ctx_slab {
+    static constexpr bool value = false;
+};
+template <class Ctx>
+struct ctx_slab<Ctx, decltype((void)Ctx::kSlab)> {
+    static constexpr bool value = Ctx::kSlab;
+};
+F3D_HD bool march_slab_near(const TerrainDev &T, const RayCtx &r) { return (f_abs(r.o.x) <= T.slab_far_x) & (f_abs(r.o.z) <= T.slab_far_z) & (r.c2 >= 0.0f); }
+F3D_HD bool march_slab_rejects(const RayCtx &r, const SlabRec &rec, float x_corner, float z_corner, float t0, float t1) {
+    const float g0 = f_fma(-rec.b, f_fma(t0, r.d.z, r.o.z) - z_corner, f_fma(-rec.a, f_fma(t0, r.d.x, r.o.x) - x_corner, f_fma(t0, r.d.y, r.o.y)));
+    const float g1 = f_fma(-rec.b, f_fma(t1, r.d.z, r.o.z) - z_corner, f_fma(-rec.a, f_fma(t1, r.d.x, r.o.x) - x_corner, f_fma(t1, r.d.y, r.o.y)));
+    return (g0 > rec.hi) & (g1 > rec.hi);
 }
 
 #ifndef F3D_LEAF_FIFO
@@ -57,6 +72,7 @@
 #if !defined(F3D_NO_BAND_PREFETCH)
     float band_mn, band_mx;
     float mesh_mn, mesh_mx;
+    float slab_a, slab_b, slab_hi;
 #endif
 };
 
@@ -73,6 +89,14 @@
         const NodeRec mesh = T.mesh_bands[band_offset + (m.nz << band_shift) + m.nx];
         m.mesh_mn = mesh.mn;
         m.mesh_mx = mesh.mx;
+    }
+    if constexpr (ctx_slab<Ctx>::value && !FUSE) {
+        if (T.slabs != nullptr && m.level > 0u) {
+            const SlabRec rec = T.slabs[band_offset - T.band_offset[1] + (m.nz << band_shift) + m.nx];
+            m.slab_a = rec.a;
+            m.slab_b = rec.b;
+            m.slab_hi = rec.hi;
+        }
     }
 #else
     static_assert(!FUSE, "the fused mesh band rides with the band prefetch");
@@ -150,7 +174,21 @@
 #endif
         const bool terrain_pass = !(lo > hi) & !march_band_rejects<CURVED>(r, lo, hi, band.mn, band.mx);
         const bool mesh_pass = FUSE ? (!(lo > hi) & !march_band_rejects<false>(r, lo, hi, m.mesh_mn, m.mesh_mx)) : false;
-        const bool pass = terrain_pass | mesh_pass;
+        bool pass = terrain_pass | mesh_pass;
+        if constexpr (ctx_slab<Ctx>::value && !FUSE) {
+            if (T.slabs != nullptr && pass && level > 0u) {
+#if !defined(F3D_NO_BAND_PREFETCH)
+                const SlabRec rec{m.slab_a, m.slab_b, 0.0f, m.slab_hi};
+#else
+                uint32_t slab_offset, slab_shift;
+                ctx.band_entry(T, level, slab_offset, slab_shift);
+                const SlabRec rec = T.slabs[slab_offset - T.band_offset[1] + (nz << slab_shift) + nx];
+#endif
+                const bool skip = march_slab_near(T, r) & march_slab_rejects(r, rec, plane_at(T.origin_x, cx0, T.spacing_x), plane_at(T.origin_z, cz0, T.spacing_z), lo, hi);
+                ctx.note(skip ? -2 : -3);
+                pass = !skip;
+            }
+        }
         if (pass) ctx.note(-1);
 #if defined(F3D_BRANCHLESS_STEP)
         {
diff --git a/forge3d_amd/csrc/f3d_scene.h b/forge3d_amd/csrc/f3d_scene.h
--- a/forge3d_amd/csrc/f3d_scene.h
+++ b/forge3d_amd/csrc/f3d_scene.h
@@ -21,6 +21,9 @@
 };
 struct alignas(8) NodeRec {
     float mn, mx;
+};
+struct alignas(16) SlabRec {
+    float a, b, lo, hi;
 };
 
 F3D_HD uint32_t child_group_index(uint32_t px, uint32_t py, uint32_t tiles_x) {
@@ -54,6 +57,8 @@
     const float4 *mesh_cell_tris;
     float mesh_top;
     uint32_t mesh_reserved;
+    const SlabRec *slabs;
+    float slab_far_x, slab_far_z;
 };
 
 struct BvhNode {
diff --git a/forge3d_amd/csrc/f3d_setup.h b/forge3d_amd/csrc/f3d_setup.h
--- a/forge3d_amd/csrc/f3d_setup.h
+++ b/forge3d_amd/csrc/f3d_setup.h
@@ -295,6 +295,28 @@
     return b;
 }
 
+inline uint64_t slab_count(const TableLayout &t) { return t.levels > 1u ? t.band_count - t.band_offset[1] : 0u; }
+inline bool slab_buildable(const TableLayout &t) { return t.levels > 1u && t.levels <= 14u; }
+inline SlabBuildParams slab_build_params(const TableLayout &t, uint32_t l, const TerrainDev &T, const LeafRec *leaves, const NodeRec *bands,
+                                         SlabRec *slabs) {
+    SlabBuildParams b{};
+    b.leaves = leaves;
+    b.leaf_tiles_x = t.tiles_x[0];
+    b.band = bands + t.band_offset[l];
+    b.dst = slabs + (t.band_offset[l] - t.band_offset[1]);
+    b.level = l;
+    b.width = t.level_w[l];
+    b.height = t.band_rows[l];
+    b.shift = t.band_shift[l];
+    b.cell_w = t.cell_w;
+    b.cell_h = t.cell_h;
+    b.spacing_x = T.spacing_x;
+    b.spacing_z = T.spacing_z;
+    b.reach_x = slab_reach(T.origin_x, t.cell_w, T.spacing_x);
+    b.reach_z = slab_reach(T.origin_z, t.cell_h, T.spacing_z);
+    return b;
+}
+
 inline PyramidBuildParams leaf_build_params(const TableLayout &t, const float *heights, uint32_t w, uint32_t h,
                                             float exaggeration, LeafRec *leaves) {
     PyramidBuildParams b{};
diff --git a/forge3d_amd/session.py b/forge3d_amd/session.py
--- a/forge3d_amd/session.py
+++ b/forge3d_amd/session.py
@@ -730,6 +730,9 @@
             raise RuntimeError("f3d_session_certificates failed")
         return {"sun_clear": int(out[0]), "primary_start": int(out[1])}
 
+    def node_slab_bytes(self) -> int:
+        return int(self._lib.f3d_session_node_slab_bytes(self._handle))
+
     def sky_blocks(self) -> dict:
         out = (C.c_uint32 * 4)()
         if self._lib.f3d_session_sky_blocks(self._handle, out) != 0:
diff --git a/include/f3d_terrain_pt.h b/include/f3d_terrain_pt.h
--- a/include/f3d_terrain_pt.h
+++ b/include/f3d_terrain_pt.h
@@ -159,6 +159,7 @@
 int f3d_session_render(f3d_session *session, f3d_terrain_ref_out *out, char *err, size_t errlen);
 int f3d_session_certificates(f3d_session *session, uint64_t out[2]);
 int f3d_session_sky_blocks(f3d_session *session, uint32_t out[4]);
+uint64_t f3d_session_node_slab_bytes(const f3d_session *session);
 typedef struct f3d_session_reaim_desc {
     uint32_t struct_size;
     float cam_origin[3], cam_look_at[3], cam_up[3];
@@ -452,6 +453,9 @@
 int f3d_build_minmax_mips(const float *heights, uint32_t width, uint32_t height, float *levels_out,
                           uint32_t *dims_out, uint32_t max_levels, uint64_t *total_floats, char *err,
                           size_t errlen);
+int f3d_build_node_slabs(const float *heights, uint32_t width, uint32_t height, float origin_x, float origin_z,
+                         float spacing_x, float spacing_z, float exaggeration, float *records_out, uint64_t capacity,
+                         uint64_t *count, char *err, size_t errlen);
 int f3d_terrain_trace_batch(const float *heights, uint32_t width, uint32_t height, float origin_x,
                             float origin_z, float spacing_x, float spacing_z, float exaggeration,
                             float inv_two_r_prime, uint32_t curvature_enabled, const float *rays,
```

Result: faster. 11820, median of 6 (+23.6%).
